# TinfoilHat0/Defending-Against-Backdoors-with-Robust-Learning-Rate

Measured on NVIDIA H100. Metric: fl_rounds_per_sec, higher is better.
Workload: dtype bf16

## Files before the change

defending-against-backdoors-with-robust-learning-rate_b200/models/native.py:

```python
from __future__ import annotations

import math
import os

import torch
import torch.nn.functional as F

from .. import ops
from .graph import FlatLayout

ACT = torch.bfloat16
FUSE_DROPOUT = bool(int(os.environ.get("RLR_FUSE_DROPOUT", "1")))
FUSE_RELU_POOL = bool(int(os.environ.get("RLR_FUSE_RELU_POOL", "1")))
EPILOGUE_BN_STATS = bool(int(os.environ.get("RLR_EPILOGUE_BN_STATS", "0")))
FWD_BRANCH = bool(int(os.environ.get("RLR_FWD_BRANCH", "1")))
BWD_BRANCH = bool(int(os.environ.get("RLR_BWD_BRANCH", "1")))
EPI_STAT_SLOTS = min(16, max(1, int(os.environ.get("RLR_EPI_STAT_SLOTS", "2"))))
FWD_SLOTS = BWD_SLOTS = max(1, int(os.environ.get("RLR_BN_SLOTS", "1")))
WGRAD_OVERLAP = bool(int(os.environ.get("RLR_WGRAD_OVERLAP", "1")))


def dropout_stream_base(seed: int, agent_id: int, rnd: int) -> int:
    z = (int(seed) * 0x9E3779B97F4A7C15 + (int(agent_id) + 1) * 0xBF58476D1CE4E5B9 + (int(rnd) + 1) * 0x94D049BB133111EB) & (2 ** 64 - 1)
    z = ((z ^ (z >> 30)) * 0xBF58476D1CE4E5B9) & (2 ** 64 - 1)
    z = ((z ^ (z >> 27)) * 0x94D049BB133111EB) & (2 ** 64 - 1)
    return (z ^ (z >> 31)) & (2 ** 62 - 1)


def native_supported(layout: FlatLayout) -> bool:
    return all(nd.op in ("conv", "bn", "gn", "relu", "maxpool", "avgpool", "flatten", "dropout", "linear", "save", "add")
               for nd in layout.nodes)


class _Op:
    __slots__ = ("kind", "node", "name", "attrs", "x", "y", "res", "relu", "saved", "acc_dx", "need_dx", "in_shape", "out_shape")

    def __init__(self, kind, **kw):
        self.kind = kind
        self.node = self.name = self.x = self.y = self.res = None
        self.attrs, self.relu, self.saved, self.acc_dx, self.need_dx = {}, False, {}, False, True
        self.in_shape = self.out_shape = None
        for k, v in kw.items():
            setattr(self, k, v)


class NativeNet:
    def __init__(self, layout: FlatLayout, device, max_batch: int, impl: str | dict = "auto", seed: int = 0, act_dtype=None):
        self.layout, self.device, self.max_batch = layout, torch.device(device), int(max_batch)
        self.act_dtype = act_dtype or ACT
        default = ("sm100" if self.device.type == "cuda" else "aten") if impl == "auto" else impl
        self.impl = dict(conv_fwd=default, conv_dgrad=default, conv_wgrad=default, bn=default, pool=default,
                         linear=default, dropout=default) if not isinstance(impl, dict) else dict(impl)
        self.seed = seed
        self.fuse_bn_stats = False
        self.first_wait = None
        self.after_first_op = None
        self.step_counter = torch.zeros(1, dtype=torch.int64, device=device)
        self._build_plan()
        self._alloc()

    def _build_plan(self):
        nodes = self.layout.nodes
        C, H, W = self.layout.in_shape
        shape = {"x": (H, W, C)}
        ver = {"x": 0}
        tid = lambda s: f"{s}@{ver[s]}"
        self.tshape = {tid("x"): shape["x"]}
        plan, consumed = [], set()
        pending_bn = {}
        alias = {}

        def new_out(slot, shp):
            ver[slot] = ver.get(slot, -1) + 1
            shape[slot] = shp
            self.tshape[tid(slot)] = shp
            return tid(slot)

        def next_same_slot(i, slot):
            for j in range(i + 1, len(nodes)):
                if j in consumed:
                    continue
                nd = nodes[j]
                if nd.op == "save":
                    if nd.inp == slot:
                        return None, None
                    continue
                if nd.inp == slot or nd.out == slot:
                    return j, nd
            return None, None

        for i, nd in enumerate(nodes):
            if i in consumed:
                continue
            a = nd.attrs
            if nd.op == "save":
                ver[nd.out] = ver.get(nd.out, -1) + 1
                alias[f"{nd.out}@{ver[nd.out]}"] = tid(nd.inp)
                shape[nd.out] = shape[nd.inp]
                self.tshape[f"{nd.out}@{ver[nd.out]}"] = shape[nd.inp]
                continue
            src = alias.get(tid(nd.inp), tid(nd.inp))
            if nd.op == "conv":
                h, w, c = shape[nd.inp]
                k, s, p = a["k"], a.get("stride", 1), a.get("pad", 0)
                ho, wo = (h + 2 * p - k) // s + 1, (w + 2 * p - k) // s + 1
                op = _Op("conv", node=i, name=nd.name, attrs=a, x=src, in_shape=(h, w, c), out_shape=(ho, wo, a["cout"]))
                j, nx = next_same_slot(i, nd.out)
                want_stats = nx is not None and nx.op == "bn"
                if nx is not None and nx.op == "relu":
                    op.relu = True
                    consumed.add(j)
                op.saved["want_stats"] = want_stats
                op.y = new_out(nd.out, op.out_shape)
                plan.append(op)
            elif nd.op in ("bn", "gn"):
                shp = shape[nd.inp]
                op = _Op(nd.op, node=i, name=nd.name, attrs=a, x=src, in_shape=shp, out_shape=shp)
                j, nx = next_same_slot(i, nd.out)
                if nx is not None and nx.op == "relu":
                    op.relu = True
                    consumed.add(j)
                    op.y = new_out(nd.out, shp)
                    plan.append(op)
                elif nx is not None and nx.op == "add":
                    pending_bn[j] = op
                else:
                    op.y = new_out(nd.out, shp)
                    plan.append(op)
            elif nd.op == "add":
                other = alias.get(tid(a["other"]), tid(a["other"]))
                op = pending_bn.pop(i, None)
                if op is None:
                    raise NotImplementedError("add without a preceding BatchNorm / GroupNorm is not used by any model in the zoo")
                op.res = other
                j, nx = next_same_slot(i, nd.out)
                if nx is not None and nx.op == "relu":
                    op.relu = True
                    consumed.add(j)
                op.y = new_out(nd.out, op.out_shape)
                plan.append(op)
            elif nd.op == "relu":
                raise NotImplementedError("stand-alone ReLU (every ReLU in the zoo follows conv/bn/linear)")
            elif nd.op == "maxpool":
                h, w, c = shape[nd.inp]
                op = _Op("maxpool", node=i, x=src, in_shape=(h, w, c), out_shape=(h // 2, w // 2, c))
                op.y = new_out(nd.out, op.out_shape)
                plan.append(op)
            elif nd.op == "avgpool":
                h, w, c = shape[nd.inp]
                op = _Op("avgpool", node=i, x=src, in_shape=(h, w, c), out_shape=(1, 1, c))
                op.y = new_out(nd.out, op.out_shape)
                plan.append(op)
            elif nd.op == "flatten":
                shp = shape[nd.inp]
                ver[nd.out] += 1
                alias[tid(nd.out)] = src
                shape[nd.out] = (int(math.prod(shp)),)
                self.tshape[tid(nd.out)] = shape[nd.out]
            elif nd.op == "dropout":
                shp = shape[nd.inp]
                prod = next((q for q in reversed(plan) if q.y == src), None)
                fusable = (prod is not None and a.get("p", 0.0) > 0 and "drop" not in prod.saved and
                           (prod.kind == "maxpool" or
                            (prod.kind == "linear" and prod.relu and ops.linear_fused_dropout_ok(prod.attrs["cout"], prod.attrs["cin"]))))
                if fusable and FUSE_DROPOUT:
                    prod.saved["drop"] = (float(a["p"]), i)
                    ver[nd.out] += 1
                    alias[tid(nd.out)] = src
                    shape[nd.out] = shp
                    self.tshape[tid(nd.out)] = shp
                else:
                    op = _Op("dropout", node=i, attrs=a, x=src, in_shape=shp, out_shape=shp)
                    op.y = new_out(nd.out, shp)
                    plan.append(op)
            elif nd.op == "linear":
                op = _Op("linear", node=i, name=nd.name, attrs=a, x=src, in_shape=shape[nd.inp], out_shape=(a["cout"],))
                j, nx = next_same_slot(i, nd.out)
                if nx is not None and nx.op == "relu":
                    op.relu = True
                    consumed.add(j)
                op.y = new_out(nd.out, op.out_shape)
                plan.append(op)
            else:
                raise NotImplementedError(nd.op)
        for op in plan:
            if op.kind != "maxpool":
                continue
            prod = next((q for q in plan if q.y == op.x), None)
            users = [q for q in plan if q.x == op.x or q.res == op.x]
            if prod is not None and prod.kind == "conv" and prod.relu and len(users) == 1 and FUSE_RELU_POOL:
                op.saved["relu_bwd_here"] = True
                prod.saved["relu_bwd_fused"] = True
        self.plan = plan
        self.alias = alias
        self.out_tid = alias.get(tid("x"), tid("x"))
        self.in_tid = "x@0"
        written = set()
        for op in reversed(plan):
            op.need_dx = op.x != self.in_tid
            if op.res is not None:
                written.add(op.res)
            if op.need_dx:
                op.acc_dx = op.x in written
                written.add(op.x)

    def _numel(self, shp):
        return int(math.prod(shp))

    def _alloc(self):
        B, dev = self.max_batch, self.device
        self.act, self.grad = {}, {}
        for op in self.plan:
            self.act[op.y] = torch.empty((B, *op.out_shape), dtype=self.act_dtype, device=dev)
        for op in self.plan:
            for t in (op.x, op.res):
                if t is not None and t != self.in_tid and t not in self.grad:
                    self.grad[t] = torch.empty((B, *self.tshape[t]), dtype=self.act_dtype, device=dev)
        self.grad[self.out_tid] = torch.empty((B, *self.tshape[self.out_tid]), dtype=self.act_dtype, device=dev)
        self.logits = torch.empty((B, self.tshape[self.out_tid][-1]), dtype=torch.float32, device=dev)
        need = [op for op in self.plan if op.kind == "bn" or (op.kind == "conv" and op.saved.get("want_stats"))]
        S = ops.STAT_SLOTS
        tot = sum(2 * op.out_shape[-1] for op in need)
        self.stats_arena = torch.zeros(max(1, tot * S), dtype=torch.float32, device=dev)
        D = BWD_SLOTS
        self.dsum_arena = torch.zeros(max(1, tot * D), dtype=torch.float32, device=dev)
        off = 0
        for op in need:
            c = op.out_shape[-1]
            op.saved["stats"] = self.stats_arena[off * S:(off + 2 * c) * S].view(S, 2, c)
            op.saved["dsum"] = self.dsum_arena[off * D:(off + 2 * c) * D].view(D, 2, c)
            op.saved["mean_rstd"] = torch.zeros(2, c, dtype=torch.float32, device=dev)
            off += 2 * c
        for op in self.plan:
            if op.kind == "gn":
                op.saved["mean_rstd"] = torch.zeros(B, 2, op.attrs["groups"], dtype=torch.float32, device=dev)
            if op.kind == "maxpool":
                op.saved["idx"] = torch.empty((B, *op.out_shape), dtype=torch.uint8, device=dev)
                if "drop" in op.saved and self.impl["pool"] != "sm100":
                    op.saved["dmask"] = torch.ones((B, *op.out_shape), dtype=torch.uint8, device=dev)
            if op.kind == "dropout":
                op.saved["mask"] = torch.empty((B, *op.out_shape), dtype=torch.uint8, device=dev)
        self._bn_src = {}
        for i, op in enumerate(self.plan):
            if not (FWD_BRANCH and op.kind == "conv" and ".downsample." in (op.name or "")):
                continue
            nxt = self.plan[i + 1] if i + 1 < len(self.plan) else None
            first = next((q for q in self.plan[:i] if q.x == op.x and q is not op), None)
            join = next((q for q in self.plan[i + 1:] if nxt is not None and q.res == nxt.y), None)
            if nxt is None or nxt.kind not in ("bn", "gn") or nxt.x != op.y or first is None or join is None:
                continue
            first.saved["fork_before"] = True
            op.saved["side_branch"] = nxt.saved["side_branch"] = True
            join.saved["join_before"] = True
        for i, op in enumerate(self.plan):
            if op.kind == "bn":
                prod = next((q for q in self.plan[:i] if q.y == op.x and q.kind == "conv"), None)
                op.saved["producer"] = prod

    def bind(self, w, wb, g, w_buffers=None):
        self.w, self.wb, self.g = w, wb, g
        lay = self.layout
        self.pw = {p.name: lay.view(w, p) for p in lay.params}
        self.pw.update({b.name: lay.view(w if w_buffers is None else w_buffers, b) for b in lay.buffers})
        self.pwb = {p.name: lay.view(wb, p) for p in lay.params} if wb is not None else {}
        self.pg = {p.name: lay.view(g, p) for p in lay.params} if g is not None else {}

    def T(self, t, B):
        return self.act[t][:B] if t != self.in_tid else self._x

    def stem_geometry(self):
        op = self.plan[0]
        if op.kind != "conv" or op.x != self.in_tid or self.impl["conv_fwd"] != "sm100" or self.impl["conv_wgrad"] != "sm100":
            return None
        return ops.stem_geometry(op.in_shape, op.attrs)

    def G(self, t, B):
        return self.grad[t][:B]

    def forward(self, x_nhwc, train: bool):
        out = self.forward_raw(x_nhwc, train)
        B = out.shape[0]
        self.logits[:B].copy_(out)
        return self.logits[:B]

    def forward_raw(self, x_nhwc, train: bool):
        B = x_nhwc.shape[0] if x_nhwc.dim() == 4 else x_nhwc.shape[0] // (self.plan[0].out_shape[0] * self.plan[0].out_shape[1])
        self._x, self._B, self._train = x_nhwc, B, train
        self._epoch = getattr(self, "_epoch", 0) + 1
        if train:
            ops.zero_(self.stats_arena)
        branch = FWD_BRANCH and self.device.type == "cuda" and ops.nn.USE_STRIDED_TMA and self.impl["conv_fwd"] == "sm100"
        if branch and getattr(self, "_branch_stream", None) is None:
            self._branch_stream = torch.cuda.Stream(self.device)
        for i, op in enumerate(self.plan):
            if branch and op.saved.get("fork_before"):
                self._branch_stream.wait_stream(torch.cuda.current_stream(self.device))
            if branch and op.saved.get("join_before"):
                torch.cuda.current_stream(self.device).wait_stream(self._branch_stream)
            if branch and op.saved.get("side_branch"):
                with torch.cuda.stream(self._branch_stream):
                    getattr(self, "_fwd_" + op.kind)(op, B, train)
            else:
                getattr(self, "_fwd_" + op.kind)(op, B, train)
            if i == 0 and self.after_first_op is not None:
                self.after_first_op()
        return self.T(self.out_tid, B).reshape(B, -1)

    def dlogits_buffer(self, B):
        return self.G(self.out_tid, B).reshape(B, -1)

    def backward(self, dlogits):
        B = dlogits.shape[0]
        gout = self.G(self.out_tid, B)
        if dlogits.data_ptr() != gout.data_ptr():
            gout.copy_(dlogits.reshape(gout.shape))
        ops.zero_(self.g)
        ops.zero_(self.dsum_arena)
        self._side = None
        if WGRAD_OVERLAP and self.device.type == "cuda":
            if getattr(self, "_side_stream", None) is None:
                self._side_stream = torch.cuda.Stream(self.device)
            self._side = self._side_stream
            self._side.wait_stream(torch.cuda.current_stream(self.device))
        branch = (BWD_BRANCH and FWD_BRANCH and self.device.type == "cuda" and ops.nn.USE_STRIDED_TMA and self.impl["conv_fwd"] == "sm100"
                  and getattr(self, "_branch_stream", None) is not None)
        cur = torch.cuda.current_stream(self.device) if branch else None
        for op in reversed(self.plan):
            if branch and op.saved.get("fork_before"):
                cur.wait_stream(self._branch_stream)
            if branch and op.saved.get("side_branch"):
                if op.kind in ("bn", "gn"):
                    self._branch_stream.wait_stream(cur)
                with torch.cuda.stream(self._branch_stream):
                    getattr(self, "_bwd_" + op.kind)(op, B)
            else:
                getattr(self, "_bwd_" + op.kind)(op, B)
        if self._side is not None:
            torch.cuda.current_stream(self.device).wait_stream(self._side)
            self._side = None

    def _epilogue_stats_free(self, op):
        if not EPILOGUE_BN_STATS or self.impl["conv_fwd"] != "sm100":
            return False
        a = op.attrs
        return a.get("stride", 1) == 1 and a["cin"] % 64 == 0 and a["cout"] % 64 == 0 and not (a["k"] == 3 and a["cin"] == 64)

    def _fwd_conv(self, op, B, train):
        a = op.attrs
        x, y = self.T(op.x, B), self.T(op.y, B)
        bias = self.pw.get(op.name + ".bias")
        stats = op.saved.get("stats") if (train and op.saved.get("want_stats") and (self.fuse_bn_stats or self._epilogue_stats_free(op))) else None
        op.saved["stats_done"] = stats is not None
        if self.impl["conv_fwd"] == "sm100" and ops.conv_supported(op.in_shape, a, "fwd"):
            ops.conv2d_fwd_sm100(x, self.pwb[op.name + ".weight"], bias, y, a.get("stride", 1), a.get("pad", 0), op.relu, stats, tag=(id(self), op.name),
                                 zero_stats=False, s2d_epoch=self._epoch, wait=self.first_wait if (op is self.plan[0] and x.dim() == 2) else None)
            return
        if self.impl["conv_fwd"] == "sm100":
            ops.note_fallback("conv_fwd", f"{op.name} in={op.in_shape} {a}")
        wt = self.pwb[op.name + ".weight"].permute(0, 3, 1, 2)
        out = F.conv2d(x.permute(0, 3, 1, 2), wt, bias.to(self.act_dtype) if bias is not None else None, a.get("stride", 1), a.get("pad", 0))
        if op.relu:
            out = F.relu(out)
        y.copy_(out.permute(0, 2, 3, 1))
        if stats is not None:
            yf = y.float().reshape(-1, y.shape[-1])
            stats[0, 0].copy_(yf.sum(0)); stats[0, 1].copy_((yf * yf).sum(0))

    def _bwd_conv(self, op, B):
        a = op.attrs
        x, y, dy = self.T(op.x, B), self.T(op.y, B), self.G(op.y, B)
        if op.relu and not op.saved.get("relu_bwd_fused"):
            ops.relu_bwd_(dy, y, self.impl["bn"])
        name = op.name + ".weight"
        gw, gb = self.pg[name], self.pg.get(op.name + ".bias")
        s, p = a.get("stride", 1), a.get("pad", 0)
        if self.impl["conv_wgrad"] == "sm100" and ops.conv_supported(op.in_shape, a, "wgrad"):
            if getattr(self, "_side", None) is not None:
                self._side.wait_stream(torch.cuda.current_stream(self.device))
                with torch.cuda.stream(self._side):
                    ops.conv2d_wgrad_sm100(x, dy, gw, gb, s, p, tag=(id(self), op.name), zero=False)
            else:
                ops.conv2d_wgrad_sm100(x, dy, gw, gb, s, p, tag=(id(self), op.name), zero=False)
        else:
            if self.impl["conv_wgrad"] == "sm100":
                ops.note_fallback("conv_wgrad", f"{op.name} in={op.in_shape} {a}")
            _, dw, db = torch.ops.aten.convolution_backward(
                dy.permute(0, 3, 1, 2), x.permute(0, 3, 1, 2), self.pwb[name].permute(0, 3, 1, 2),
                [a["cout"]] if gb is not None else None, [s, s], [p, p], [1, 1], False, [0, 0], 1, [False, True, gb is not None])
            gw.copy_(dw.permute(0, 2, 3, 1))
            if gb is not None:
                gb.copy_(db)
        if not op.need_dx:
            return
        dx = self.G(op.x, B)
        if self.impl["conv_dgrad"] == "sm100" and ops.conv_supported(op.in_shape, a, "dgrad"):
            ops.conv2d_dgrad_sm100(dy, self.pwb[name], dx, s, p, op.acc_dx)
            return
        if self.impl["conv_dgrad"] == "sm100":
            ops.note_fallback("conv_dgrad", f"{op.name} in={op.in_shape} {a}")
        di, _, _ = torch.ops.aten.convolution_backward(
            dy.permute(0, 3, 1, 2), x.permute(0, 3, 1, 2), self.pwb[name].permute(0, 3, 1, 2), None, [s, s], [p, p], [1, 1],
            False, [0, 0], 1, [True, False, False])
        di = di.permute(0, 2, 3, 1)
        if op.acc_dx:
            dx.add_(di)
        else:
            dx.copy_(di)

    def _fwd_bn(self, op, B, train):
        a = op.attrs
        x, y = self.T(op.x, B), self.T(op.y, B)
        res = self.T(op.res, B) if op.res is not None else None
        gamma, beta = self.pw[op.name + ".weight"], self.pw[op.name + ".bias"]
        rm, rv = self.pw[op.name + ".running_mean"], self.pw[op.name + ".running_var"]
        prod = op.saved["producer"]
        stats = prod.saved["stats"] if (train and prod is not None and prod.saved.get("stats_done")) else None
        if stats is not None and not self.fuse_bn_stats:
            stats = stats[0:EPI_STAT_SLOTS]
        count = x.numel() // x.shape[-1]
        ops.bn_fwd(x, y, res, gamma, beta, rm, rv, stats, op.saved["mean_rstd"], count, a.get("eps", 1e-5),
                   a.get("momentum", 0.1), train, op.relu, self.impl["bn"],
                   stats_buf=op.saved["stats"][0:FWD_SLOTS] if train else None)

    def _bwd_bn(self, op, B):
        x, y, dy = self.T(op.x, B), self.T(op.y, B), self.G(op.y, B)
        dres = self.G(op.res, B) if op.res is not None else None
        dx = self.G(op.x, B)
        gamma = self.pw[op.name + ".weight"]
        ops.bn_bwd(dy, y, x, gamma, op.saved["mean_rstd"], op.saved["dsum"], dx, dres,
                   self.pg[op.name + ".weight"], self.pg[op.name + ".bias"], op.relu, self.impl["bn"], zero_dsum=False,
                   beta=self.pw[op.name + ".bias"])

    def _fwd_gn(self, op, B, train):
        a = op.attrs
        res = self.T(op.res, B) if op.res is not None else None
        ops.gn_fwd(self.T(op.x, B), self.T(op.y, B), res, self.pw[op.name + ".weight"], self.pw[op.name + ".bias"],
                   op.saved["mean_rstd"][:B], a["groups"], a.get("eps", 1e-5), op.relu, self.impl["bn"])

    def _bwd_gn(self, op, B):
        dres = self.G(op.res, B) if op.res is not None else None
        ops.gn_bwd(self.G(op.y, B), self.T(op.y, B), self.T(op.x, B), self.pw[op.name + ".weight"], op.saved["mean_rstd"][:B],
                   self.G(op.x, B), dres, self.pg[op.name + ".weight"], self.pg[op.name + ".bias"], op.attrs["groups"], op.relu,
                   self.impl["bn"], zero=False)

    def _drop(self, op, train=True):
        d = op.saved.get("drop")
        return (d[0], self.seed, self.step_counter, d[1]) if (d is not None and train) else None

    def _fwd_maxpool(self, op, B, train):
        drop = self._drop(op, train)
        op.saved["drop_on"] = drop is not None
        mask = op.saved["dmask"][:B] if (drop is not None and "dmask" in op.saved) else None
        ops.maxpool2_fwd(self.T(op.x, B), self.T(op.y, B), op.saved["idx"][:B], self.impl["pool"], drop, mask)

    def _bwd_maxpool(self, op, B):
        drop = self._drop(op, op.saved.get("drop_on", False))
        mask = op.saved["dmask"][:B] if (drop is not None and "dmask" in op.saved) else None
        ops.maxpool2_bwd(self.G(op.y, B), op.saved["idx"][:B], self.G(op.x, B), self.impl["pool"], drop, mask,
                         relu_out=self.T(op.y, B) if op.saved.get("relu_bwd_here") else None)

    def _fwd_avgpool(self, op, B, train):
        ops.avgpool_fwd(self.T(op.x, B), self.T(op.y, B), self.impl["pool"])

    def _bwd_avgpool(self, op, B):
        ops.avgpool_bwd(self.G(op.y, B), self.G(op.x, B), self.impl["pool"])

    def _fwd_dropout(self, op, B, train):
        x, y = self.T(op.x, B), self.T(op.y, B)
        if not train:
            y.copy_(x.reshape(y.shape))
            return
        ops.dropout_fwd(x.reshape(B, -1), y.reshape(B, -1), op.saved["mask"][:B].reshape(B, -1), op.attrs["p"], self.seed,
                        self.step_counter, op.node, self.impl["dropout"])

    def _bwd_dropout(self, op, B):
        ops.dropout_bwd(self.G(op.y, B).reshape(B, -1), op.saved["mask"][:B].reshape(B, -1), self.G(op.x, B).reshape(B, -1),
                        op.attrs["p"], self.impl["dropout"])

    def _fwd_linear(self, op, B, train):
        x, y = self.T(op.x, B).reshape(B, -1), self.T(op.y, B)
        drop = self._drop(op, train)
        op.saved["drop_on"] = drop is not None
        ops.linear_fwd(x, self.pwb[op.name + ".weight"], self.pw.get(op.name + ".bias"), y, op.relu, self.impl["linear"], drop)

    def _bwd_linear(self, op, B):
        x, y, dy = self.T(op.x, B).reshape(B, -1), self.T(op.y, B), self.G(op.y, B)
        if op.relu:
            scale = 1.0 / (1.0 - op.saved["drop"][0]) if op.saved.get("drop_on", False) else 1.0
            ops.relu_bwd_(dy, y, self.impl["bn"], scale)
        dx = self.G(op.x, B).reshape(B, -1) if op.need_dx else None
        ops.linear_bwd(x, dy, self.pwb[op.name + ".weight"], dx, self.pg[op.name + ".weight"], self.pg.get(op.name + ".bias"),
                       op.acc_dx, self.impl["linear"], zero=False)


class NativeTrainer:
    name = "native"

    def __init__(self, layout, args, device, max_shard: int, impl="auto"):
        self.layout, self.args = layout, args
        self.device = torch.device(device)
        assert self.device.type == "cuda", "the native trainer runs on sm_90a devices only"
        n = layout.n_total
        self.w = torch.zeros(n, dtype=torch.float32, device=device)
        self.wb = torch.zeros(n, dtype=torch.bfloat16, device=device)
        self.g = torch.zeros(n, dtype=torch.float32, device=device)
        self.m = torch.zeros(n, dtype=torch.float32, device=device)
        self.bs = args.bs
        self.net = NativeNet(layout, device, self.bs, impl, seed=args.seed)
        self.net.bind(self.w, self.wb, self.g)
        self.opt = ops.FlatSGD(n, device, args.client_lr, args.client_moment, 10.0, args.clip, n_pgd=layout.n_vote)
        self.loss_sum = torch.zeros(1, dtype=torch.float32, device=device)
        self.use_graphs = not args.no_graphs
        self.max_shard = max_shard
        self.perm = torch.zeros(max(1, max_shard), dtype=torch.int64, device=device)
        self.cursor = torch.zeros(1, dtype=torch.int32, device=device)
        self.y = torch.zeros(self.bs, dtype=torch.int64, device=device)
        C, H, W = layout.in_shape
        self.x = torch.zeros(self.bs, H, W, C, dtype=ACT, device=device)
        self.stem = self.net.stem_geometry()
        self.xA = torch.zeros(self.bs * self.stem[2] * self.stem[3], 64, dtype=ACT, device=device) if self.stem else None
        self._graphs = {}
        self._eval_nets = {}
        self.bcast = None

    def attach_broadcast(self, fused):
        if self.stem is None or fused.w_bf16 is None:
            return False
        self.bcast = fused
        return True

    def _bind_first(self, w0):
        f = self.bcast
        self.net.bind(f.w_global, f.w_bf16, self.g, w_buffers=self.w)
        lay = self.layout
        first_w = lay.by_name[self.net.plan[0].name + ".weight"]
        lo, hi = f.slices_of(first_w.offset, first_w.offset + first_w.numel)
        self.net.first_wait = (f.ready_ptr, lo, hi, f.epoch_dev) if f.ready_ptr else None
        tail_src, tail_dst = f.w_global[lay.n_vote:], self.w[lay.n_vote:]
        self.net.after_first_op = lambda: ops.ext().acquire_slices(f.ready_ptr, 0, max(0, f.n_slices - 1), f.epoch_dev, tail_src, tail_dst)

    def _bind_normal(self):
        self.net.bind(self.w, self.wb, self.g)
        self.net.first_wait = None
        self.net.after_first_op = None

    def _step(self, dataset, B, w0, first=False):
        if first:
            self._bind_first(w0)
        meta = dataset.meta
        if self.stem is not None:
            k, pad, Ho, Wo = self.stem
            xin = self.xA[:B * Ho * Wo]
            ops.gather_im2col(dataset.data, self.perm, meta.mean, meta.std, k, pad, xin, cursor=self.cursor, targets=dataset.targets,
                              out_labels=self.y, batch=B)
        else:
            xin = self.x[:B]
            ops.gather_normalize(dataset.data, self.perm, meta.mean, meta.std, out=xin, nhwc=True, cursor=self.cursor,
                                 targets=dataset.targets, out_labels=self.y, batch=B)
        logits = self.net.forward_raw(xin, True)
        _, dl = ops.softmax_xent(logits, self.y[:B], True, self.loss_sum, dlogits=self.net.dlogits_buffer(B))
        self.net.backward(dl)
        self.opt.step(self.w, self.g, self.m, w0=w0, w_bf16=self.wb, w_in=self.bcast.w_global if first else None)
        ops.ext().advance_cursor(self.cursor, B, self.net.step_counter)
        if first:
            self._bind_normal()

    def _get_graph(self, dataset, B, w0, first=False):
        key = (B, dataset.data.data_ptr(), w0.data_ptr(), bool(first))
        if key in self._graphs:
            return self._graphs[key]
        keep = (self.w.clone(), self.wb.clone(), self.m.clone(), self.cursor.clone(), self.loss_sum.clone(),
                self.net.step_counter.clone())
        self.perm.zero_()
        s = torch.cuda.Stream(self.device)
        s.wait_stream(torch.cuda.current_stream(self.device))
        with torch.cuda.stream(s):
            for _ in range(3):
                self.cursor.zero_()
                c0 = ops.launch_calls()
                self._step(dataset, B, w0, first)
                self._launches = ops.launch_calls() - c0
        torch.cuda.current_stream(self.device).wait_stream(s)
        self.cursor.zero_()
        graph = torch.cuda.CUDAGraph()
        with torch.cuda.graph(graph, capture_error_mode="thread_local"):
            self._step(dataset, B, w0, first)
        self.w.copy_(keep[0]); self.wb.copy_(keep[1]); self.m.copy_(keep[2]); self.cursor.copy_(keep[3])
        self.loss_sum.copy_(keep[4]); self.net.step_counter.copy_(keep[5])
        self._graphs[key] = graph
        return graph

    def train_agent(self, agent, w_global, out, rnd: int = 0):
        args, bs = self.args, self.bs
        dataset, n = agent.dataset, agent.n_data
        self.loss_sum.zero_()
        graphs = self.use_graphs and n <= self.max_shard
        fused = self.bcast is not None and w_global.data_ptr() == self.bcast.w_global.data_ptr()
        if graphs:
            full = self._get_graph(dataset, bs, w_global) if n >= bs else None
            tail = self._get_graph(dataset, n % bs, w_global) if n % bs else None
            if fused:
                first_g = self._get_graph(dataset, bs if n >= bs else n % bs, w_global, first=True)
        if not fused:
            ops.round_init(w_global, self.w, self.wb, self.m)
        self.net.step_counter.fill_(dropout_stream_base(args.seed, agent.id, rnd))
        steps = 0
        for ep in range(args.local_ep):
            idx = agent.epoch_indices(args.seed, rnd, ep)
            self.perm[:n].copy_(idx)
            self.cursor.zero_()
            for b in range(n // bs):
                is_first = fused and ep == 0 and b == 0
                if graphs:
                    (first_g if is_first else full).replay()
                else:
                    self._step(dataset, bs, w_global, first=is_first)
            if n % bs:
                is_first = fused and ep == 0 and n < bs
                if graphs:
                    (first_g if is_first else tail).replay()
                else:
                    self._step(dataset, n % bs, w_global, first=is_first)
            steps += (n + bs - 1) // bs
        if out.data_ptr() != self.w.data_ptr():
            out.copy_(self.w)
        return {"loss_sum": self.loss_sum, "steps": steps}

    def launches_per_step(self):
        return getattr(self, "_launches", 0)

    @torch.no_grad()
    def eval_forward(self, w):
        key = w.data_ptr()
        if key not in self._eval_nets:
            net = NativeNet(self.layout, self.device, self.bs, self.net.impl, seed=self.args.seed)
            self._eval_nets = {key: (net, torch.zeros(self.layout.n_total, dtype=ACT, device=self.device))}
        net, wb = self._eval_nets[key]
        wb.copy_(w)
        net.bind(w, wb, None)

        def fwd(x_nchw):
            x = x_nchw.permute(0, 2, 3, 1).to(ACT).contiguous()
            return net.forward(x, False).clone()
        return fwd
```

defending-against-backdoors-with-robust-learning-rate_b200/ops/csrc/gemm.cu:

```cuda
#include <cuda.h>
#include <stdlib.h>

#include "common.cuh"
#include "gemm.h"
#include "stem_gather.cuh"
#include "wgmma.cuh"

namespace rlr {

using namespace wg;

constexpr int BM = 128;
constexpr int BK = 64;
constexpr int kConsumers = 256;
constexpr int kThreads = kConsumers + 64;
constexpr int kEpiThreads = kConsumers;

template <int BN, int kOcc = 2>
struct TileCfg {
    static constexpr int kStages = kOcc == 3 ? (BN == 64 ? 3 : 2) : (BN == 64 ? 4 : 3);
    static constexpr int kABytes = BM * BK * 2;
    static constexpr int kBBytes = BN * BK * 2;
    static constexpr int kStageBytes = kABytes + kBBytes;
    static constexpr int kPitch = BN * 2 + 16;
    static constexpr int kStagingBytes = BM * kPitch;
    static constexpr int kRingBytes = kStages * kStageBytes;
    static_assert(kStagingBytes + 2 * BN * 4 <= kRingBytes, "staging aliases the operand ring");
    static constexpr int kTailBytes = BN == 128 ? 2048 : 1024;
    static constexpr int kSmemBytes = kRingBytes + 1024  + kTailBytes;
};

struct __align__(8) SharedTail {
    uint64_t full[4];
    uint64_t empty[4];
    uint64_t pad0;
    uint32_t pad1;
    uint32_t pad2;
    int row_index[BM];
};
static_assert(sizeof(SharedTail) <= 640, "the bias slice starts 640 bytes into the tail");

template <int BN, bool kStats, bool kBMN, int kOcc = 2>
__global__ void __launch_bounds__(kThreads, kOcc)
umma_conv_gemm_kernel(const __grid_constant__ CUtensorMap tmA, const __grid_constant__ CUtensorMap tmB, const __grid_constant__ CUtensorMap tmC,
                       const ConvGemmParams p) {
    using Cfg = TileCfg<BN, kOcc>;
    extern __shared__ uint8_t smem_raw[];
    uint8_t* smem = reinterpret_cast<uint8_t*>((reinterpret_cast<uintptr_t>(smem_raw) + 1023) & ~uintptr_t(1023));
    SharedTail* tail = reinterpret_cast<SharedTail*>(smem + Cfg::kRingBytes);

    const int warp = threadIdx.x >> 5, lane = threadIdx.x & 31;
    const int tile_m = blockIdx.x, tile_n = blockIdx.y;
    long long* dbg = p.dbg ? p.dbg + ((size_t)blockIdx.y * gridDim.x + blockIdx.x) * 8 : nullptr;
    if (dbg && threadIdx.x == 0) { dbg[0] = (long long)gtimer(); uint32_t sm; asm volatile("mov.u32 %0, %%smid;" : "=r"(sm)); dbg[7] = sm; }

    int n0 = 0, h0 = 0, w0 = 0;
    if (p.mode == 1) {
        const int tw_i = tile_m % p.tiles_w;
        const int th_i = (tile_m / p.tiles_w) % p.tiles_h;
        const int tn_i = tile_m / (p.tiles_w * p.tiles_h);
        w0 = tw_i * p.TW; h0 = th_i * p.TH; n0 = tn_i * p.TN;
    }

    if (warp == 8 && lane == 0) {
        prefetch_tmap(&tmA);
        prefetch_tmap(&tmB);
        if (p.tma_store) prefetch_tmap(&tmC);
        for (int s = 0; s < Cfg::kStages; ++s) { mbar_init(&tail->full[s], (p.split_prod || p.b_src) ? 2 : 1); mbar_init(&tail->empty[s], 8); }
        fence_barrier_init();
    }
    if (threadIdx.x < BM) {
        const int r = threadIdx.x;
        int gi;
        if (p.mode == 1) {
            const int tw = r % p.TW, th = (r / p.TW) % p.TH, tn = r / (p.TW * p.TH);
            const int w = w0 + tw, h = h0 + th, n = n0 + tn;
            gi = (w < p.Wo && h < p.Ho && n < p.NB) ? ((n * p.OutH + h * p.out_stride + p.out_ph) * p.OutW + w * p.out_stride + p.out_pw) : -1;
        } else {
            gi = tile_m * BM + r;
            if (gi >= p.M) gi = -1;
        }
        tail->row_index[r] = gi;
    }
    __syncthreads();
    pdl_wait();
    pdl_trigger();
    if (dbg && threadIdx.x == 0) dbg[1] = (long long)gtimer();

    if (warp == 8) {
        if (p.b_src) {
            if (lane == 0) {
                mbar_expect_tx(&tail->full[0], Cfg::kABytes);
                tma_load_2d(&tmA, &tail->full[0], smem, 0, tile_m * BM);
            }
            stem_gather_b(p, smem + Cfg::kABytes, BN, tile_n, lane);
            if (lane == 0) mbar_arrive(&tail->full[0]);
        } else if (lane == 0) {
            int stage = 0;
            uint32_t phase = 0;
            for (int kb = 0; kb < p.num_kb; ++kb) {
                mbar_wait(&tail->empty[stage], phase ^ 1);
                uint8_t* sa = smem + stage * Cfg::kStageBytes;
                uint8_t* sb = sa + Cfg::kABytes;
                mbar_expect_tx(&tail->full[stage], p.split_prod ? Cfg::kABytes : Cfg::kStageBytes);
                if (dbg && kb == 0) dbg[2] = (long long)gtimer();
                if (p.mode == 1) {
                    const int tap = kb / p.cblocks, cb = kb - tap * p.cblocks;
                    tma_load_4d(&tmA, &tail->full[stage], sa, cb * BK, w0 * p.in_stride + p.dw[tap], h0 * p.in_stride + p.dh[tap],
                                n0 + p.dn[tap]);
                } else {
                    tma_load_2d(&tmA, &tail->full[stage], sa, kb * BK, tile_m * BM);
                }
                if (p.split_prod) {
                } else if (kBMN) {
                    const int tap = kb / p.cblocks, cb = kb - tap * p.cblocks;
                    for (int g = 0; g < BN / 64; ++g)
                        tma_load_2d(&tmB, &tail->full[stage], sb + g * 8192, p.wtap[tap] * p.wcols + tile_n * BN + g * 64, cb * BK);
                } else {
                    tma_load_2d(&tmB, &tail->full[stage], sb, kb * BK, tile_n * BN);
                }
                if (++stage == Cfg::kStages) { stage = 0; phase ^= 1; }
            }
        }
    } else if (warp == 9) {
        if (p.split_prod && lane == 0) {
            int stage = 0;
            uint32_t phase = 0;
            for (int kb = 0; kb < p.num_kb; ++kb) {
                mbar_wait(&tail->empty[stage], phase ^ 1);
                uint8_t* sb = smem + stage * Cfg::kStageBytes + Cfg::kABytes;
                mbar_expect_tx(&tail->full[stage], Cfg::kBBytes);
                if (kBMN) {
                    const int tap = kb / p.cblocks, cb = kb - tap * p.cblocks;
                    for (int g = 0; g < BN / 64; ++g)
                        tma_load_2d(&tmB, &tail->full[stage], sb + g * 8192, p.wtap[tap] * p.wcols + tile_n * BN + g * 64, cb * BK);
                } else {
                    tma_load_2d(&tmB, &tail->full[stage], sb, kb * BK, tile_n * BN);
                }
                if (++stage == Cfg::kStages) { stage = 0; phase ^= 1; }
            }
        }
    } else {
        const int et = threadIdx.x;
        const int wgi = et >> 7, t = et & 127;
        const int col0 = tile_n * BN;
        const bool has_bias = !kBMN && p.bias != nullptr;
        float* bias_w = reinterpret_cast<float*>(reinterpret_cast<uint8_t*>(tail) + 640);
        if (has_bias)
            for (int i = et; i < BN; i += kEpiThreads) bias_w[i] = (col0 + i < p.N) ? p.bias[col0 + i] : 0.f;
        float acc[BN / 2];
#pragma unroll
        for (int i = 0; i < BN / 2; ++i) acc[i] = 0.f;
        {
            int stage = 0;
            uint32_t phase = 0;
            consumer_mainloop<BN, Cfg::kStages, Cfg::kStageBytes, Cfg::kABytes, kBMN>(
                acc, smem, tail->full, tail->empty, p.num_kb, (uint32_t)wgi * 64 * 128, p.b_src ? smem_u32(smem + Cfg::kABytes) : 0u,
                stage, phase, lane);
        }
        if (dbg && et == 0) dbg[4] = (long long)gtimer();
        named_bar(1, kEpiThreads);
        if (dbg && et == 0) dbg[5] = (long long)gtimer();
        const float* bias_s = bias_w;
        uint8_t* staging = smem;
        float* red = reinterpret_cast<float*>(staging + Cfg::kStagingBytes);
        const int r0 = wgi * 64 + frag_row(t, 0);
        int gi_r[2];
        gi_r[0] = tail->row_index[r0];
        gi_r[1] = tail->row_index[r0 + 8];
        if (kStats) {
            for (int i = et; i < 2 * BN; i += kEpiThreads) red[i] = 0.f;
            named_bar(1, kEpiThreads);
        }
        const bool tma_out = !kStats && p.tma_store;
#pragma unroll
        for (int j = 0; j < BN / 8; ++j) {
            const int c = frag_col(t, 4 * j);
            float s1[2] = {0.f, 0.f}, s2[2] = {0.f, 0.f};
#pragma unroll
            for (int h = 0; h < 2; ++h) {
                const int row = r0 + 8 * h, gi_row = gi_r[h];
                float a = acc[4 * j + 2 * h], b = acc[4 * j + 2 * h + 1];
                if (has_bias) { a += bias_s[c]; b += bias_s[c + 1]; }
                if (p.relu) { a = fmaxf(a, 0.f); b = fmaxf(b, 0.f); }
                if (p.drop.thr) {
                    const uint32_t keep8 = dropout_keep8(p.drop, ((long long)(gi_row < 0 ? 0 : gi_row) * p.ldc + col0 + 8 * j) >> 3);
                    a = (keep8 >> (c & 7) & 1) ? a * p.drop.scale : 0.f;
                    b = (keep8 >> ((c & 7) + 1) & 1) ? b * p.drop.scale : 0.f;
                }
                const uint32_t packed = pack_bf16x2(a, b);
                if (kStats && gi_row >= 0) {
                    const float2 rq = __bfloat1622float2(*reinterpret_cast<const __nv_bfloat162*>(&packed));
                    s1[0] += rq.x; s1[1] += rq.y; s2[0] += rq.x * rq.x; s2[1] += rq.y * rq.y;
                }
                if (tma_out)
                    *reinterpret_cast<uint32_t*>(staging + (c >> 6) * (BM * 128) + row * 128 + ((((c & 63) >> 3) ^ (row & 7)) << 4) + (c & 7) * 2) = packed;
                else
                    *reinterpret_cast<uint32_t*>(staging + row * Cfg::kPitch + c * 2) = packed;
            }
            if (kStats) {
#pragma unroll
                for (int o = 4; o < 32; o <<= 1)
#pragma unroll
                    for (int e = 0; e < 2; ++e) {
                        s1[e] += __shfl_xor_sync(0xffffffffu, s1[e], o);
                        s2[e] += __shfl_xor_sync(0xffffffffu, s2[e], o);
                    }
                if (lane < 4) {
                    atomicAdd(&red[c], s1[0]); atomicAdd(&red[c + 1], s1[1]);
                    atomicAdd(&red[BN + c], s2[0]); atomicAdd(&red[BN + c + 1], s2[1]);
                }
            }
        }
        if (tma_out) {
            fence_proxy_async_smem();
            named_bar(1, kEpiThreads);
            if (dbg && et == 0) dbg[6] = (long long)gtimer();
            if (et == 0) {
#pragma unroll
                for (int g = 0; g < BN / 64; ++g) {
                    if (col0 + g * 64 >= p.N) break;
                    if (p.mode == 1) tma_store_4d(&tmC, staging + g * (BM * 128), col0 + g * 64, w0, h0, n0);
                    else tma_store_2d(&tmC, staging + g * (BM * 128), col0 + g * 64, tile_m * BM);
                }
                tma_store_commit();
            }
            if (p.stats) {
                constexpr int kPerCol = kEpiThreads / BN, kRows = BM / kPerCol;
                const int c = et % BN;
                const int r_lo = (et / BN) * kRows, r_hi = r_lo + kRows;
                const uint8_t* colp = staging + (c >> 6) * (BM * 128) + (c & 7) * 2;
                const int chunk = (c & 63) >> 3;
                float s1 = 0.f, s2 = 0.f;
#pragma unroll 8
                for (int r = r_lo; r < r_hi; ++r) {
                    if (tail->row_index[r] < 0) continue;
                    const float v = __bfloat162float(*reinterpret_cast<const __nv_bfloat16*>(colp + r * 128 + ((chunk ^ (r & 7)) << 4)));
                    s1 += v; s2 += v * v;
                }
                if (col0 + c < p.N) {
                    float* dst = p.stats + (size_t)(blockIdx.x % p.stat_slots) * 2 * p.N + col0 + c;
                    atomicAdd(dst, s1);
                    atomicAdd(dst + p.N, s2);
                }
            }
            if (et == 0) tma_store_wait_read();
        } else {
        named_bar(1, kEpiThreads);
        if (dbg && et == 0) dbg[6] = (long long)gtimer();
        constexpr int kChunks = BN * 2 / 16;
        __nv_bfloat16* out = reinterpret_cast<__nv_bfloat16*>(p.out);
        constexpr int kIters = BM * kChunks / kEpiThreads;
        constexpr int kBatch = kIters < 8 ? kIters : 8;
#pragma unroll
        for (int it0 = 0; it0 < kIters; it0 += kBatch) {
            uint4 oldv[kBatch];
            if (p.accumulate) {
#pragma unroll
                for (int j = 0; j < kBatch; ++j) {
                    const int idx = et + (it0 + j) * kEpiThreads, r = idx / kChunks, ch = idx - r * kChunks;
                    const int gi = tail->row_index[r];
                    oldv[j] = make_uint4(0, 0, 0, 0);
                    if (gi >= 0 && col0 + ch * 8 < p.N) oldv[j] = *reinterpret_cast<const uint4*>(out + (size_t)gi * p.ldc + col0 + ch * 8);
                }
            }
#pragma unroll
            for (int j = 0; j < kBatch; ++j) {
                const int idx = et + (it0 + j) * kEpiThreads, r = idx / kChunks, ch = idx - r * kChunks;
                const int gi = tail->row_index[r];
                if (gi < 0 || col0 + ch * 8 >= p.N) continue;
                uint4 val = *reinterpret_cast<const uint4*>(staging + r * Cfg::kPitch + ch * 16);
                if (p.accumulate) {
                    const __nv_bfloat162* o2 = reinterpret_cast<const __nv_bfloat162*>(&oldv[j]);
                    __nv_bfloat162* v2 = reinterpret_cast<__nv_bfloat162*>(&val);
#pragma unroll
                    for (int q = 0; q < 4; ++q) {
                        const float2 a = __bfloat1622float2(v2[q]), b = __bfloat1622float2(o2[q]);
                        v2[q] = __floats2bfloat162_rn(a.x + b.x, a.y + b.y);
                    }
                }
                *reinterpret_cast<uint4*>(out + (size_t)gi * p.ldc + col0 + ch * 8) = val;
            }
        }
        if (kStats) {
            named_bar(1, kEpiThreads);
            for (int i = et; i < 2 * BN; i += kEpiThreads)
                if (col0 + (i % BN) < p.N)
                    atomicAdd(p.stats + (size_t)(blockIdx.x % kStatSlots) * 2 * p.N + (i < BN ? 0 : p.N) + col0 + (i % BN), red[i]);
        }
        }
    }
}

typedef CUresult (*EncodeTiledFn)(CUtensorMap*, CUtensorMapDataType, cuuint32_t, void*, const cuuint64_t*, const cuuint64_t*,
                                  const cuuint32_t*, const cuuint32_t*, CUtensorMapInterleave, CUtensorMapSwizzle,
                                  CUtensorMapL2promotion, CUtensorMapFloatOOBfill);

static EncodeTiledFn get_encode_fn() {
    static EncodeTiledFn fn = nullptr;
    if (!fn) {
        void* f = nullptr;
        cudaDriverEntryPointQueryResult q;
        if (cudaGetDriverEntryPoint("cuTensorMapEncodeTiled", &f, cudaEnableDefault, &q) != cudaSuccess || !f) return nullptr;
        fn = reinterpret_cast<EncodeTiledFn>(f);
    }
    return fn;
}

cudaError_t make_tmap_bf16(CUtensorMap* map, const void* base, int rank, const uint64_t* dims, const uint64_t* strides_bytes,
                           const uint32_t* box, const uint32_t* elem_strides = nullptr) {
    EncodeTiledFn fn = get_encode_fn();
    if (!fn) return cudaErrorNotSupported;
    cuuint64_t gd[5], gs[4];
    cuuint32_t bx[5], es[5];
    for (int i = 0; i < rank; ++i) {
        gd[i] = dims[i];
        es[i] = elem_strides ? elem_strides[i] : 1;
        bx[i] = box[i] * es[i];
        if (bx[i] > 256 || es[i] < 1 || es[i] > 8) return cudaErrorInvalidValue;
    }
    for (int i = 0; i + 1 < rank; ++i) gs[i] = strides_bytes[i];
    const CUresult r = fn(map, CU_TENSOR_MAP_DATA_TYPE_BFLOAT16, (cuuint32_t)rank, const_cast<void*>(base), gd, gs, bx, es,
                          CU_TENSOR_MAP_INTERLEAVE_NONE, CU_TENSOR_MAP_SWIZZLE_128B, CU_TENSOR_MAP_L2_PROMOTION_L2_256B,
                          CU_TENSOR_MAP_FLOAT_OOB_FILL_NONE);
    return r == CUDA_SUCCESS ? cudaSuccess : cudaErrorInvalidValue;
}

template <int BN>
cudaError_t launch_persistent_bn(const CUtensorMap& tmA, const CUtensorMap& tmB, const ConvGemmParams& p, int m_tiles, int num_sms,
                                 cudaStream_t st, int occ = 1);

static int g_occ3 = -1;
void set_conv_occ3(int level) { g_occ3 = level < 0 ? 0 : (level > 1 ? 1 : level); }
static int conv_occ3() {
    if (g_occ3 < 0) { const char* e = getenv("RLR_CONV_OCC3"); set_conv_occ3(e ? atoi(e) : 1); }
    return g_occ3;
}

template <int BN>
static cudaError_t launch_bn_occ3(const CUtensorMap& tmA, const CUtensorMap& tmB, const CUtensorMap& tmC, const ConvGemmParams& p, int m_tiles,
                                  cudaStream_t st) {
    using Cfg = TileCfg<BN, 3>;
    static bool configured = false;
    if (!configured) {
        RLR_CUDA_CHECK(cudaFuncSetAttribute(umma_conv_gemm_kernel<BN, false, false, 3>, cudaFuncAttributeMaxDynamicSharedMemorySize, Cfg::kSmemBytes));
        RLR_CUDA_CHECK(cudaFuncSetAttribute(umma_conv_gemm_kernel<BN, false, true, 3>, cudaFuncAttributeMaxDynamicSharedMemorySize, Cfg::kSmemBytes));
        configured = true;
    }
    dim3 grid(m_tiles, (p.N + BN - 1) / BN);
    if (p.b_mn) return launch_kernel(umma_conv_gemm_kernel<BN, false, true, 3>, grid, dim3(kThreads), Cfg::kSmemBytes, st, tmA, tmB, tmC, p);
    return launch_kernel(umma_conv_gemm_kernel<BN, false, false, 3>, grid, dim3(kThreads), Cfg::kSmemBytes, st, tmA, tmB, tmC, p);
}

static int sm_count() {
    static const int sms = [] {
        int dev = 0, n = 0;
        if (cudaGetDevice(&dev) != cudaSuccess || cudaDeviceGetAttribute(&n, cudaDevAttrMultiProcessorCount, dev) != cudaSuccess) return 132;
        return n;
    }();
    return sms;
}

static int g_persistent = -1;
void set_persistent_conv(int on) { g_persistent = on ? 1 : 0; }

static int persistent_sms() {
    if (g_persistent < 0) { const char* e = getenv("RLR_PERSISTENT_CONV"); g_persistent = (e && atoi(e) > 0) ? 1 : 0; }
    if (!g_persistent) return 0;
    static const int sms = [] {
        int dev = 0, n = 0;
        if (cudaGetDevice(&dev) != cudaSuccess || cudaDeviceGetAttribute(&n, cudaDevAttrMultiProcessorCount, dev) != cudaSuccess) return 0;
        return n;
    }();
    return sms;
}

static int g_split_prod = -1;
void set_conv_split_producer(int on) { g_split_prod = on ? 1 : 0; }
static long long* g_trace = nullptr;
void set_conv_trace(long long* buf) { g_trace = buf; }
long long* conv_trace_buf() { return g_trace; }

static int g_tma_store = -1;
void set_conv_tma_store(int on) { g_tma_store = on ? 1 : 0; }
static bool tma_store_enabled() {
    if (g_tma_store < 0) { const char* e = getenv("RLR_TMA_STORE"); g_tma_store = (e && atoi(e) == 0) ? 0 : 1; }
    return g_tma_store != 0;
}
static cudaError_t make_out_tmap(CUtensorMap* tmC, const ConvGemmParams& p) {
    if (p.ldc % 8) return cudaErrorInvalidValue;
    if (p.mode == 1) {
        const uint64_t d[4] = {(uint64_t)p.N, (uint64_t)p.Wo, (uint64_t)p.Ho, (uint64_t)p.NB};
        const uint64_t s[3] = {(uint64_t)p.out_stride * p.ldc * 2, (uint64_t)p.out_stride * p.OutW * p.ldc * 2, (uint64_t)p.OutH * p.OutW * p.ldc * 2};
        const uint32_t b[4] = {64, (uint32_t)p.TW, (uint32_t)p.TH, (uint32_t)p.TN};
        const char* base = reinterpret_cast<const char*>(p.out) + ((size_t)p.out_ph * p.OutW + p.out_pw) * p.ldc * 2;
        return make_tmap_bf16(tmC, base, 4, d, s, b);
    }
    const uint64_t d[2] = {(uint64_t)p.N, (uint64_t)p.M}, s[1] = {(uint64_t)p.ldc * 2};
    const uint32_t b[2] = {64, BM};
    return make_tmap_bf16(tmC, p.out, 2, d, s, b);
}

template <int BN>
static cudaError_t launch_bn(const CUtensorMap& tmA, const CUtensorMap& tmB, const ConvGemmParams& p_in, int m_tiles, cudaStream_t st) {
    using Cfg = TileCfg<BN>;
    ConvGemmParams p = p_in;
    p.dbg = g_trace;
    CUtensorMap tmC = tmA;
    {
        static const int epi_slots = [] { const char* e = getenv("RLR_EPI_STAT_SLOTS"); int v = e ? atoi(e) : 2; return v < 1 ? 1 : (v > kStatSlots ? kStatSlots : v); }();
        p.stat_slots = epi_slots;
    }
    p.tma_store = 0;
    if (tma_store_enabled() && !p.accumulate && ((reinterpret_cast<uintptr_t>(p.out) & 15) == 0) && make_out_tmap(&tmC, p) == cudaSuccess)
        p.tma_store = 1;
    if (g_split_prod < 0) { const char* e = getenv("RLR_SPLIT_PRODUCER"); g_split_prod = (e && atoi(e) == 0) ? 0 : 1; }
    p.split_prod = (g_split_prod && !p.b_src) ? 1 : 0;
    if (p.b_src && !p.stats && p.N <= BN) {
        static const int stem_persistent = [] { const char* e = getenv("RLR_STEM_PERSISTENT"); return e ? atoi(e) : 2; }();
        if (stem_persistent && m_tiles >= 2 * sm_count())
            return launch_persistent_bn<BN>(tmA, tmB, p, m_tiles, sm_count(), st, stem_persistent == 2 ? 2 : 1);
    }
    if (!p.stats && !p.b_src && persistent_sms() > 0 && m_tiles * ((p.N + BN - 1) / BN) > persistent_sms())
        return launch_persistent_bn<BN>(tmA, tmB, p, m_tiles, persistent_sms(), st);
    if constexpr (BN == 64)
        if ((!p.stats || p.tma_store) && conv_occ3() >= 1) return launch_bn_occ3<BN>(tmA, tmB, tmC, p, m_tiles, st);
    static bool configured = false;
    if (!configured) {
        RLR_CUDA_CHECK(cudaFuncSetAttribute(umma_conv_gemm_kernel<BN, false, false>, cudaFuncAttributeMaxDynamicSharedMemorySize, Cfg::kSmemBytes));
        RLR_CUDA_CHECK(cudaFuncSetAttribute(umma_conv_gemm_kernel<BN, true, false>, cudaFuncAttributeMaxDynamicSharedMemorySize, Cfg::kSmemBytes));
        RLR_CUDA_CHECK(cudaFuncSetAttribute(umma_conv_gemm_kernel<BN, false, true>, cudaFuncAttributeMaxDynamicSharedMemorySize, Cfg::kSmemBytes));
        configured = true;
    }
    dim3 grid(m_tiles, (p.N + BN - 1) / BN);
    if (p.b_mn) return launch_kernel(umma_conv_gemm_kernel<BN, false, true>, grid, dim3(kThreads), Cfg::kSmemBytes, st, tmA, tmB, tmC, p);
    if (p.stats && !p.tma_store) return launch_kernel(umma_conv_gemm_kernel<BN, true, false>, grid, dim3(kThreads), Cfg::kSmemBytes, st, tmA, tmB, tmC, p);
    return launch_kernel(umma_conv_gemm_kernel<BN, false, false>, grid, dim3(kThreads), Cfg::kSmemBytes, st, tmA, tmB, tmC, p);
}

static int pick_bn(int N) { return (N % 128 == 0) ? 128 : 64; }

cudaError_t launch_gemm_bf16(const void* A, const void* B, void* out, int M, int N, int K, int lda, int ldb, int ldc,
                             const float* bias, int relu, int accumulate, float* stats, cudaStream_t st, const DropSpec* drop) {
    if (K % BK || N % 8 || M <= 0) return cudaErrorInvalidValue;
    if (drop && drop->thr && (accumulate || stats || ldc % 8)) return cudaErrorInvalidValue;
    const int m_tiles = (M + BM - 1) / BM;
    int bn = pick_bn(N);
    {
        static const int small64 = [] { const char* e = getenv("RLR_GEMM_SMALL_BN64"); return e ? atoi(e) : 0; }();
        if (small64 && bn == 128 && m_tiles * (N / 128) < sm_count()) bn = 64;
    }
    CUtensorMap tmA, tmB;
    {
        const uint64_t d[2] = {(uint64_t)K, (uint64_t)M}, s[1] = {(uint64_t)lda * 2};
        const uint32_t b[2] = {BK, BM};
        RLR_CUDA_CHECK(make_tmap_bf16(&tmA, A, 2, d, s, b));
    }
    {
        const uint64_t d[2] = {(uint64_t)K, (uint64_t)N}, s[1] = {(uint64_t)ldb * 2};
        const uint32_t b[2] = {BK, (uint32_t)bn};
        RLR_CUDA_CHECK(make_tmap_bf16(&tmB, B, 2, d, s, b));
    }
    ConvGemmParams p{};
    p.M = M; p.N = N; p.num_kb = K / BK; p.mode = 0; p.in_stride = 1; p.out_stride = 1;
    p.out = out; p.ldc = ldc; p.bias = bias; p.stats = stats; p.relu = relu; p.accumulate = accumulate;
    if (drop && drop->thr) p.drop = *drop;
    return bn == 128 ? launch_bn<128>(tmA, tmB, p, m_tiles, st) : launch_bn<64>(tmA, tmB, p, m_tiles, st);
}

cudaError_t launch_stem_gemm_bf16(const void* A, const void* W, void* out, int M, int N, int kvalid, int ldw, const float* bias, int relu,
                                  float* stats, const uint32_t* wait_flags, int wait_lo, int wait_hi, const uint32_t* wait_epoch,
                                  cudaStream_t st) {
    if (N % 8 || M <= 0 || kvalid < 1 || kvalid > BK || ldw < kvalid) return cudaErrorInvalidValue;
    if (wait_flags && (!wait_epoch || wait_lo > wait_hi || wait_lo < 0)) return cudaErrorInvalidValue;
    const int m_tiles = (M + BM - 1) / BM;
    const int bn = pick_bn(N);
    CUtensorMap tmA;
    {
        const uint64_t d[2] = {(uint64_t)BK, (uint64_t)M}, s[1] = {(uint64_t)BK * 2};
        const uint32_t b[2] = {BK, BM};
        RLR_CUDA_CHECK(make_tmap_bf16(&tmA, A, 2, d, s, b));
    }
    ConvGemmParams p{};
    p.M = M; p.N = N; p.num_kb = 1; p.mode = 0; p.in_stride = 1; p.out_stride = 1;
    p.out = out; p.ldc = N; p.bias = bias; p.stats = stats; p.relu = relu; p.accumulate = 0;
    p.b_src = reinterpret_cast<const __nv_bfloat16*>(W); p.b_ld = ldw; p.b_kvalid = kvalid;
    p.wait_flags = wait_flags; p.wait_lo = wait_lo; p.wait_hi = wait_hi; p.wait_epoch = wait_epoch;
    return bn == 128 ? launch_bn<128>(tmA, tmA, p, m_tiles, st) : launch_bn<64>(tmA, tmA, p, m_tiles, st);
}

static int pow2_ceil(int x) { int p = 1; while (p < x) p <<= 1; return p; }

cudaError_t launch_conv_bf16(const void* x, const void* w, void* out, int NB, int planes, int Hin, int Win, int Cin, int Ho, int Wo,
                             int Cout, int ldc, int ntaps, const int* dh, const int* dw, const int* dplane, const float* bias,
                             int relu, int accumulate, float* stats, cudaStream_t st, const int* wtap, int w_taps_total,
                             int in_stride, int out_stride, int out_ph, int out_pw) {
    if (Cin % BK || Cout % 8 || ntaps < 1 || ntaps > 9) return cudaErrorInvalidValue;
    if (in_stride < 1 || in_stride > 2 || out_stride < 1 || out_stride > 2 || (in_stride > 1 && planes != 1)) return cudaErrorInvalidValue;
    if (wtap && (stats || Cout % 64)) return cudaErrorInvalidValue;
    int bn = pick_bn(Cout);
    ConvGemmParams p{};
    {
        static const int small_bn64 = [] { const char* e = getenv("RLR_SMALL_BN64"); return e ? atoi(e) : 1; }();
        const long long px = (long long)NB * Ho * Wo;
        if (small_bn64 && bn == 128 && ((px + BM - 1) / BM) * (Cout / 128) < sm_count()) bn = 64;
    }
    int TW = pow2_ceil(Wo); if (TW > BM) TW = BM;
    int TH = pow2_ceil(Ho); if (TW * TH > BM) TH = BM / TW;
    int TN = BM / (TW * TH);
    p.TW = TW; p.TH = TH; p.TN = TN;
    p.tiles_w = (Wo + TW - 1) / TW; p.tiles_h = (Ho + TH - 1) / TH;
    const int tiles_n = (NB + TN - 1) / TN;
    const int m_tiles = p.tiles_w * p.tiles_h * tiles_n;
    p.M = NB * Ho * Wo; p.N = Cout; p.mode = 1; p.cblocks = Cin / BK; p.num_kb = ntaps * p.cblocks; p.ntaps = ntaps;
    p.Ho = Ho; p.Wo = Wo; p.NB = NB;
    p.in_stride = in_stride; p.out_stride = out_stride; p.out_ph = out_ph; p.out_pw = out_pw; p.OutH = Ho * out_stride; p.OutW = Wo * out_stride;
    for (int t = 0; t < ntaps; ++t) { p.dh[t] = (int8_t)dh[t]; p.dw[t] = (int8_t)dw[t]; p.dn[t] = dplane[t] * NB; }
    p.out = out; p.ldc = ldc; p.bias = bias; p.stats = stats; p.relu = relu; p.accumulate = accumulate;
    CUtensorMap tmA, tmB;
    {
        const uint64_t d[4] = {(uint64_t)Cin, (uint64_t)Win, (uint64_t)Hin, (uint64_t)planes * NB};
        const uint64_t s[3] = {(uint64_t)Cin * 2, (uint64_t)Win * Cin * 2, (uint64_t)Hin * Win * Cin * 2};
        const uint32_t b[4] = {BK, (uint32_t)TW, (uint32_t)TH, (uint32_t)TN};
        const uint32_t es[4] = {1, (uint32_t)in_stride, (uint32_t)in_stride, 1};
        RLR_CUDA_CHECK(make_tmap_bf16(&tmA, x, 4, d, s, b, in_stride > 1 ? es : nullptr));
    }
    if (wtap) {
        if (bias) return cudaErrorInvalidValue;
        p.b_mn = 1; p.wcols = Cout;
        for (int t = 0; t < ntaps; ++t) p.wtap[t] = wtap[t];
        const uint64_t cols = (uint64_t)w_taps_total * Cout;
        const uint64_t d[2] = {cols, (uint64_t)Cin}, s[1] = {cols * 2};
        const uint32_t b[2] = {64, BK};
        RLR_CUDA_CHECK(make_tmap_bf16(&tmB, w, 2, d, s, b));
    } else {
        const uint64_t K = (uint64_t)ntaps * Cin;
        const uint64_t d[2] = {K, (uint64_t)Cout}, s[1] = {K * 2};
        const uint32_t b[2] = {BK, (uint32_t)bn};
        RLR_CUDA_CHECK(make_tmap_bf16(&tmB, w, 2, d, s, b));
    }
    return bn == 128 ? launch_bn<128>(tmA, tmB, p, m_tiles, st) : launch_bn<64>(tmA, tmB, p, m_tiles, st);
}

}
```

defending-against-backdoors-with-robust-learning-rate_b200/ops/csrc/gemm.h:

```cpp
#pragma once
#include <cuda_runtime.h>
#include <cuda_bf16.h>
#include <stdint.h>

#include "dropspec.h"

namespace rlr {

constexpr int kStatSlots = 16;

struct ConvGemmParams {
    int M, N, num_kb;
    int mode;
    int cblocks;
    int TW, TH, TN;
    int Ho, Wo, NB;
    int tiles_w, tiles_h;
    int ntaps;
    int in_stride;
    int out_stride, out_ph, out_pw, OutH, OutW;
    int8_t dh[9], dw[9];
    int dn[9];
    int b_mn;
    int wtap[9];
    int wcols;
    DropSpec drop;
    int tma_store;
    int split_prod;
    long long* dbg;
    const __nv_bfloat16* b_src;
    int b_ld, b_kvalid;
    const uint32_t* wait_flags;
    int wait_lo, wait_hi;
    const uint32_t* wait_epoch;
    void* out;
    int ldc;
    const float* bias;
    float* stats;
    int stat_slots;
    int relu, accumulate;
};

cudaError_t launch_gemm_bf16(const void* A, const void* B, void* out, int M, int N, int K, int lda, int ldb, int ldc,
                             const float* bias, int relu, int accumulate, float* stats, cudaStream_t st, const DropSpec* drop = nullptr);
cudaError_t launch_stem_gemm_bf16(const void* A, const void* W, void* out, int M, int N, int kvalid, int ldw, const float* bias, int relu,
                                  float* stats, const uint32_t* wait_flags, int wait_lo, int wait_hi, const uint32_t* wait_epoch,
                                  cudaStream_t st);
void set_pdl(int on);
cudaError_t launch_gemm_splitk_bf16(const void* A, const void* B, void* out, float* ws, int M, int N, int K, const float* bias, int relu,
                                    int num_sms, cudaStream_t st, const DropSpec* drop = nullptr);
void set_persistent_conv(int on);
void set_conv_occ3(int level);
void set_conv_tma_store(int on);
void set_conv_split_producer(int on);
void set_conv_trace(long long* buf);
long long* conv_trace_buf();
cudaError_t launch_conv_bf16(const void* x, const void* w, void* out, int NB, int planes, int Hin, int Win, int Cin, int Ho, int Wo,
                             int Cout, int ldc, int ntaps, const int* dh, const int* dw, const int* dplane, const float* bias,
                             int relu, int accumulate, float* stats, cudaStream_t st, const int* wtap = nullptr, int w_taps_total = 0,
                             int in_stride = 1, int out_stride = 1, int out_ph = 0, int out_pw = 0);

cudaError_t launch_conv3x3_halo_bf16(const void* x, const void* w, void* out, int NB, int Hin, int Win, int H, int W, int Cout, const float* bias,
                                     int relu, int accumulate, float* stats, int bo_mode, long long* dbg, int num_sms, cudaStream_t st);

cudaError_t launch_conv3x3_halo3_bf16(const void* x, const void* w, void* out, int NB, int H, int W, int Cout, const float* bias, int relu,
                                      int accumulate, int num_sms, cudaStream_t st);

cudaError_t launch_conv_wgrad_bf16(const void* dy, const void* x, float* dW, int NB, int planes, int Hin, int Win, int Cin, int Cin_valid,
                                   int Ho, int Wo, int Cout, int ntaps, const int* dh, const int* dw, const int* dplane, int num_sms,
                                   cudaStream_t st, int in_stride = 1);
cudaError_t launch_conv_wgrad_halo_bf16(const void* dy, const void* x, float* dW, int NB, int H, int W, int Cin_valid, int Cout,
                                        int num_sms, cudaStream_t st);
cudaError_t launch_linear_wgrad_bf16(const void* dy, const void* x, float* dW, int B, int N, int K, int num_sms, cudaStream_t st);

cudaError_t launch_ordered_sum_f32(float* out, const float* part, int nparts, long long n, cudaStream_t st);
cudaError_t launch_ordered_sum_f64(double* out, const double* part, int nparts, long long n, cudaStream_t st);
cudaError_t launch_channel_stats(const __nv_bfloat16* x, long long M, int C, float* stats , int num_sms, cudaStream_t st,
                                 int only_sum = 0, int nslots = 1);
cudaError_t launch_bn_finalize(const float* stats, int slots, float* mean_rstd, float* running_mean, float* running_var, int C,
                               float count, float eps, float momentum, int train, cudaStream_t st);
cudaError_t launch_bn_apply(const __nv_bfloat16* x, const __nv_bfloat16* res, __nv_bfloat16* y, const float* gamma, const float* beta,
                            float* mean_rstd, long long M, int C, int relu, int fin_mode, const float* stats, int slots, float count,
                            float eps, float momentum, float* running_mean, float* running_var, int num_sms, cudaStream_t st);
cudaError_t launch_bn_bwd_reduce(const __nv_bfloat16* dy, const __nv_bfloat16* y, const __nv_bfloat16* x, const float* mean_rstd,
                                 float* dsum , long long M, int C, int relu, int num_sms, cudaStream_t st,
                                 const float* gamma = nullptr, const float* beta = nullptr, int nslots = 1);
cudaError_t launch_bn_bwd_apply(const __nv_bfloat16* dy, const __nv_bfloat16* y, const __nv_bfloat16* x, const float* gamma,
                                const float* mean_rstd, const float* dsum, __nv_bfloat16* dx, __nv_bfloat16* dres, float* dgamma,
                                float* dbeta, long long M, int C, int relu, int num_sms, cudaStream_t st, const float* beta = nullptr, int nslots = 1);
cudaError_t launch_gn_fwd(const __nv_bfloat16* x, const __nv_bfloat16* res, __nv_bfloat16* y, const float* gamma, const float* beta,
                          float* mean_rstd, int B, int HW, int C, int G, float eps, int relu, int num_sms, cudaStream_t st);
cudaError_t launch_gn_bwd(const __nv_bfloat16* dy, const __nv_bfloat16* y, const __nv_bfloat16* x, const float* gamma,
                          const float* mean_rstd, __nv_bfloat16* dx, __nv_bfloat16* dres, float* dgamma, float* dbeta, int B, int HW,
                          int C, int G, int relu, int num_sms, cudaStream_t st);
cudaError_t launch_relu_bwd(__nv_bfloat16* dy, const __nv_bfloat16* y, long long n, int num_sms, cudaStream_t st, float scale = 1.0f);
cudaError_t launch_maxpool2_fwd(const __nv_bfloat16* x, __nv_bfloat16* y, uint8_t* idx, int B, int H, int W, int C, cudaStream_t st,
                                float drop_p = 0.f, uint64_t seed = 0, const long long* step = nullptr, uint64_t stream = 0);
cudaError_t launch_maxpool2_bwd(const __nv_bfloat16* dy, const uint8_t* idx, __nv_bfloat16* dx, int B, int H, int W, int C, cudaStream_t st,
                                float drop_p, uint64_t seed, const long long* step, uint64_t stream, const __nv_bfloat16* zmask);
cudaError_t launch_avgpool_fwd(const __nv_bfloat16* x, __nv_bfloat16* y, int B, int HW, int C, cudaStream_t st);
cudaError_t launch_avgpool_bwd(const __nv_bfloat16* dy, __nv_bfloat16* dx, int B, int HW, int C, cudaStream_t st);
cudaError_t launch_dropout_fwd(const __nv_bfloat16* x, __nv_bfloat16* y, uint8_t* mask, long long n, float p, uint64_t seed,
                               const long long* step, uint64_t stream, cudaStream_t st);
cudaError_t launch_dropout_bwd(const __nv_bfloat16* dy, const uint8_t* mask, __nv_bfloat16* dx, long long n, float p, cudaStream_t st);
cudaError_t launch_space_to_depth(const __nv_bfloat16* x, __nv_bfloat16* y, int NB, int H, int W, int C, int num_sms, cudaStream_t st);
cudaError_t launch_im2col_small(const __nv_bfloat16* x, __nv_bfloat16* A, int NB, int H, int W, int C, int Ho, int Wo, int k, int pad,
                                int num_sms, cudaStream_t st);
cudaError_t launch_depth_to_space(const __nv_bfloat16* x4, __nv_bfloat16* y, int NB, int H, int W, int C, int accumulate, int plane_mask,
                                  int num_sms, cudaStream_t st);
cudaError_t launch_filter_gather_transpose(const __nv_bfloat16* w, __nv_bfloat16* wt, int Cout, int T, int Cin, int nsub, const int* taps,
                                           cudaStream_t st);
cudaError_t launch_filter_transpose(const __nv_bfloat16* w, __nv_bfloat16* wt, int Cout, int ntaps, int Cin, cudaStream_t st);
cudaError_t launch_linear_small_fwd(const __nv_bfloat16* x, const __nv_bfloat16* w, const float* bias, __nv_bfloat16* y, int B, int K,
                                    int N, int relu, cudaStream_t st);
cudaError_t launch_linear_small_fwd2(const __nv_bfloat16* x, const __nv_bfloat16* w, const float* bias, __nv_bfloat16* y, int B, int K,
                                     int N, int relu, cudaStream_t st);
cudaError_t launch_linear_small_bwd2(const __nv_bfloat16* x, const __nv_bfloat16* dy, const __nv_bfloat16* w, __nv_bfloat16* dx,
                                     float* dw, float* db, int B, int K, int N, int accumulate_dx, cudaStream_t st);
cudaError_t launch_linear_small_bwd(const __nv_bfloat16* x, const __nv_bfloat16* dy, const __nv_bfloat16* w, __nv_bfloat16* dx,
                                    float* dw, float* db, int B, int K, int N, int accumulate_dx, cudaStream_t st);

}
```

defending-against-backdoors-with-robust-learning-rate_b200/ops/csrc/gemm_binding.cpp:

```cpp
#include <torch/extension.h>
#include <ATen/cuda/CUDAContext.h>
#include <c10/cuda/CUDAGuard.h>
#include <c10/cuda/CUDAStream.h>
#include <c10/cuda/CUDACachingAllocator.h>

#include <vector>

#include "gemm.h"

namespace rlr {
void* scratch_alloc(size_t bytes, cudaStream_t st) {
    return c10::cuda::CUDACachingAllocator::raw_alloc_with_stream(bytes < 256 ? 256 : bytes, st);
}
void scratch_free(void* p) { c10::cuda::CUDACachingAllocator::raw_delete(p); }
}

namespace {
inline cudaStream_t cur_stream() { return c10::cuda::getCurrentCUDAStream().stream(); }
inline int num_sms() { return at::cuda::getCurrentDeviceProperties()->multiProcessorCount; }
inline void check(cudaError_t e, const char* what) { TORCH_CHECK(e == cudaSuccess, what, ": ", cudaGetErrorString(e)); }
template <typename T>
inline T* opt(const c10::optional<at::Tensor>& t) { return t.has_value() && t->defined() ? reinterpret_cast<T*>(t->data_ptr()) : nullptr; }
inline const __nv_bfloat16* bf(const at::Tensor& t) {
    TORCH_CHECK(t.is_cuda() && t.scalar_type() == at::kBFloat16 && t.is_contiguous(), "expected contiguous CUDA bf16 tensor");
    return reinterpret_cast<const __nv_bfloat16*>(t.data_ptr());
}
inline __nv_bfloat16* bfm(at::Tensor& t) { return const_cast<__nv_bfloat16*>(bf(t)); }
inline const __nv_bfloat16* bfo(const c10::optional<at::Tensor>& t) { return t.has_value() && t->defined() ? bf(*t) : nullptr; }
inline float* f32(const at::Tensor& t) {
    TORCH_CHECK(t.is_cuda() && t.scalar_type() == at::kFloat && t.is_contiguous(), "expected contiguous CUDA fp32 tensor");
    return reinterpret_cast<float*>(t.data_ptr());
}

static rlr::DropSpec drop_spec(double p, int64_t seed, const c10::optional<at::Tensor>& step, int64_t stream) {
    rlr::DropSpec d{};
    if (p > 0.0) {
        TORCH_CHECK(p < 1.0 && step.has_value() && step->defined() && step->scalar_type() == at::kLong, "fused dropout needs p < 1 and an int64 step counter");
        d.thr = (uint32_t)(p * 65536.0); d.scale = (float)(1.0 / (1.0 - p)); d.seed = (uint64_t)seed; d.stream = (uint64_t)stream;
        d.step = reinterpret_cast<const long long*>(step->data_ptr<int64_t>());
    }
    return d;
}

void gemm_bf16(at::Tensor A, at::Tensor B, at::Tensor out, c10::optional<at::Tensor> bias, bool relu, bool accumulate,
               c10::optional<at::Tensor> stats, double drop_p, int64_t drop_seed, c10::optional<at::Tensor> drop_step, int64_t drop_stream) {
    c10::cuda::CUDAGuard g(A.device());
    const rlr::DropSpec drop = drop_spec(drop_p, drop_seed, drop_step, drop_stream);
    const int M = A.size(0), K = A.size(1), N = B.size(0);
    TORCH_CHECK(B.size(1) == K && out.size(0) == M && out.size(1) == N);
    TORCH_CHECK(!stats.has_value() || !stats->defined() || stats->numel() == (int64_t)rlr::kStatSlots * 2 * N, "stats must be [STAT_SLOTS,2,N]");
    check(rlr::launch_gemm_bf16(bf(A), bf(B), bfm(out), M, N, K, K, K, N, opt<const float>(bias), relu, accumulate, opt<float>(stats),
                                cur_stream(), drop.thr ? &drop : nullptr), "gemm_bf16");
}

void stem_gemm_bf16(at::Tensor A, at::Tensor W, at::Tensor out, c10::optional<at::Tensor> bias, bool relu, c10::optional<at::Tensor> stats,
                    int64_t ready_ptr, int64_t lo, int64_t hi, c10::optional<at::Tensor> epoch) {
    c10::cuda::CUDAGuard g(A.device());
    const int M = A.size(0), N = W.size(0), kvalid = W.size(1);
    TORCH_CHECK(A.dim() == 2 && A.size(1) == 64 && W.dim() == 2 && W.is_contiguous() && out.size(0) == M && out.size(1) == N, "stem_gemm shapes");
    TORCH_CHECK(ready_ptr == 0 || (epoch.has_value() && epoch->defined() && epoch->scalar_type() == at::kInt), "epoch must be an int32 device tensor");
    check(rlr::launch_stem_gemm_bf16(bf(A), bf(W), bfm(out), M, N, kvalid, kvalid, opt<const float>(bias), relu, opt<float>(stats),
                                     reinterpret_cast<const uint32_t*>(ready_ptr), (int)lo, (int)hi,
                                     ready_ptr ? reinterpret_cast<const uint32_t*>(epoch->data_ptr()) : nullptr, cur_stream()), "stem_gemm_bf16");
}

void conv_bf16(at::Tensor x, at::Tensor w, at::Tensor out, int64_t NB, int64_t planes, std::vector<int64_t> dh, std::vector<int64_t> dw,
               std::vector<int64_t> dplane, c10::optional<at::Tensor> bias, bool relu, bool accumulate, c10::optional<at::Tensor> stats,
               std::vector<int64_t> wtap, int64_t w_taps_total) {
    c10::cuda::CUDAGuard g(x.device());
    TORCH_CHECK(x.dim() == 4 && out.dim() == 4 && w.dim() == 2);
    const int Hin = x.size(1), Win = x.size(2), Cin = x.size(3), Ho = out.size(1), Wo = out.size(2), Cout = out.size(3);
    const int T = (int)dh.size();
    const bool bmn = !wtap.empty();
    TORCH_CHECK(x.size(0) == planes * NB && out.size(0) == NB);
    TORCH_CHECK(bmn ? (w.size(0) == Cin && w.size(1) == w_taps_total * Cout && (int)wtap.size() == T)
                    : (w.size(0) == Cout && w.size(1) == (int64_t)T * Cin), "filter shape");
    TORCH_CHECK(!stats.has_value() || !stats->defined() || stats->numel() == (int64_t)rlr::kStatSlots * 2 * Cout, "stats must be [STAT_SLOTS,2,Cout]");
    int a[9], b[9], c[9], wt[9];
    for (int t = 0; t < T; ++t) { a[t] = (int)dh[t]; b[t] = (int)dw[t]; c[t] = (int)dplane[t]; wt[t] = bmn ? (int)wtap[t] : 0; }
    check(rlr::launch_conv_bf16(bf(x), bf(w), bfm(out), (int)NB, (int)planes, Hin, Win, Cin, Ho, Wo, Cout, Cout, T, a, b, c,
                                opt<const float>(bias), relu, accumulate, opt<float>(stats), cur_stream(), bmn ? wt : nullptr,
                                (int)w_taps_total), "conv_bf16");
}

void gemm_splitk_bf16(at::Tensor A, at::Tensor B, at::Tensor out, at::Tensor ws, c10::optional<at::Tensor> bias, bool relu, double drop_p,
                      int64_t drop_seed, c10::optional<at::Tensor> drop_step, int64_t drop_stream) {
    c10::cuda::CUDAGuard g(A.device());
    const rlr::DropSpec drop = drop_spec(drop_p, drop_seed, drop_step, drop_stream);
    const int M = A.size(0), K = A.size(1), N = B.size(0);
    TORCH_CHECK(B.size(1) == K && out.size(0) == M && out.size(1) == N && ws.numel() == (int64_t)M * N);
    check(rlr::launch_gemm_splitk_bf16(bf(A), bf(B), bfm(out), f32(ws), M, N, K, opt<const float>(bias), relu, num_sms(), cur_stream(),
                                       drop.thr ? &drop : nullptr), "gemm_splitk_bf16");
}

void conv_bf16_strided(at::Tensor x, at::Tensor w, at::Tensor out, std::vector<int64_t> dh, std::vector<int64_t> dw,
                       c10::optional<at::Tensor> bias, bool relu, bool accumulate, std::vector<int64_t> wtap, int64_t w_taps_total,
                       int64_t in_stride, int64_t out_stride, int64_t out_ph, int64_t out_pw) {
    c10::cuda::CUDAGuard g(x.device());
    TORCH_CHECK(x.dim() == 4 && out.dim() == 4 && w.dim() == 2 && x.size(0) == out.size(0));
    TORCH_CHECK(out.size(1) % out_stride == 0 && out.size(2) % out_stride == 0, "output image must be a multiple of out_stride");
    const int NB = x.size(0), Hin = x.size(1), Win = x.size(2), Cin = x.size(3), Cout = out.size(3);
    const int Ho = out.size(1) / out_stride, Wo = out.size(2) / out_stride;
    const int T = (int)dh.size();
    const bool bmn = !wtap.empty();
    TORCH_CHECK(bmn ? (w.size(0) == Cin && w.size(1) == w_taps_total * Cout && (int)wtap.size() == T)
                    : (w.size(0) == Cout && w.size(1) == (int64_t)T * Cin), "filter shape");
    int a[9], b[9], c[9] = {0}, wt[9];
    for (int t = 0; t < T; ++t) { a[t] = (int)dh[t]; b[t] = (int)dw[t]; wt[t] = bmn ? (int)wtap[t] : 0; }
    check(rlr::launch_conv_bf16(bf(x), bf(w), bfm(out), NB, 1, Hin, Win, Cin, Ho, Wo, Cout, Cout, T, a, b, c, opt<const float>(bias), relu,
                                accumulate, nullptr, cur_stream(), bmn ? wt : nullptr, (int)w_taps_total, (int)in_stride, (int)out_stride,
                                (int)out_ph, (int)out_pw), "conv_bf16_strided");
}

void conv3x3_halo_bf16(at::Tensor x, at::Tensor w, at::Tensor out, c10::optional<at::Tensor> bias, bool relu, bool accumulate,
                       c10::optional<at::Tensor> stats, int64_t bo_mode, c10::optional<at::Tensor> dbg) {
    c10::cuda::CUDAGuard g(x.device());
    TORCH_CHECK(x.dim() == 4 && x.size(3) == 64 && out.dim() == 4 && w.dim() == 2 && w.size(1) == 9 * 64 && w.size(0) == out.size(3));
    TORCH_CHECK(out.size(0) == x.size(0) && out.size(1) - x.size(1) == out.size(2) - x.size(2), "halo conv: output = input + 2*pad - 2, pad in {0,1,2}");
    TORCH_CHECK(!stats.has_value() || !stats->defined() || stats->numel() == (int64_t)rlr::kStatSlots * 2 * out.size(3), "stats must be [STAT_SLOTS,2,Cout]");
    check(rlr::launch_conv3x3_halo_bf16(bf(x), bf(w), bfm(out), x.size(0), x.size(1), x.size(2), out.size(1), out.size(2), out.size(3), opt<const float>(bias), relu,
                                        accumulate, opt<float>(stats), (int)bo_mode, opt<long long>(dbg), num_sms(), cur_stream()), "conv3x3_halo_bf16");
}

void conv3x3_halo3_bf16(at::Tensor x, at::Tensor w, at::Tensor out, c10::optional<at::Tensor> bias, bool relu, bool accumulate) {
    c10::cuda::CUDAGuard g(x.device());
    TORCH_CHECK(x.dim() == 4 && x.size(3) == 64 && out.dim() == 4 && w.dim() == 2 && w.size(1) == 9 * 64 && w.size(0) == out.size(3));
    TORCH_CHECK(out.size(0) == x.size(0) && out.size(1) == x.size(1) && out.size(2) == x.size(2));
    check(rlr::launch_conv3x3_halo3_bf16(bf(x), bf(w), bfm(out), x.size(0), x.size(1), x.size(2), out.size(3), opt<const float>(bias), relu,
                                         accumulate, num_sms(), cur_stream()), "conv3x3_halo3_bf16");
}

void conv_wgrad_bf16(at::Tensor dy, at::Tensor x, at::Tensor dW, int64_t NB, int64_t planes, int64_t cin_valid, std::vector<int64_t> dh,
                     std::vector<int64_t> dw, std::vector<int64_t> dplane) {
    c10::cuda::CUDAGuard g(x.device());
    TORCH_CHECK(x.dim() == 4 && dy.dim() == 4);
    const int Hin = x.size(1), Win = x.size(2), Cin = x.size(3), Ho = dy.size(1), Wo = dy.size(2), Cout = dy.size(3);
    const int T = (int)dh.size();
    TORCH_CHECK(x.size(0) == planes * NB && dy.size(0) == NB && dW.numel() == (int64_t)Cout * T * cin_valid);
    TORCH_CHECK((Cout <= 64 && Cout % 8 == 0) || Cout % 128 == 0, "wgrad: Cout must be <= 64 or a multiple of 128");
    int a[9], b[9], c[9];
    for (int t = 0; t < T; ++t) { a[t] = (int)dh[t]; b[t] = (int)dw[t]; c[t] = (int)dplane[t]; }
    check(rlr::launch_conv_wgrad_bf16(bf(dy), bf(x), f32(dW), (int)NB, (int)planes, Hin, Win, Cin, (int)cin_valid, Ho, Wo, Cout, T, a, b, c,
                                      num_sms(), cur_stream()), "conv_wgrad_bf16");
}
void conv_wgrad_bf16_strided(at::Tensor dy, at::Tensor x, at::Tensor dW, int64_t cin_valid, std::vector<int64_t> dh, std::vector<int64_t> dw,
                             int64_t in_stride) {
    c10::cuda::CUDAGuard g(x.device());
    TORCH_CHECK(x.dim() == 4 && dy.dim() == 4 && x.size(0) == dy.size(0));
    const int NB = x.size(0), Hin = x.size(1), Win = x.size(2), Cin = x.size(3), Ho = dy.size(1), Wo = dy.size(2), Cout = dy.size(3);
    const int T = (int)dh.size();
    TORCH_CHECK(dW.numel() == (int64_t)Cout * T * cin_valid);
    TORCH_CHECK((Cout <= 64 && Cout % 8 == 0) || Cout % 128 == 0, "wgrad: Cout must be <= 64 or a multiple of 128");
    int a[9], b[9], c[9] = {0};
    for (int t = 0; t < T; ++t) { a[t] = (int)dh[t]; b[t] = (int)dw[t]; }
    check(rlr::launch_conv_wgrad_bf16(bf(dy), bf(x), f32(dW), NB, 1, Hin, Win, Cin, (int)cin_valid, Ho, Wo, Cout, T, a, b, c, num_sms(),
                                      cur_stream(), (int)in_stride), "conv_wgrad_bf16_strided");
}
void conv_wgrad_halo_bf16(at::Tensor dy, at::Tensor x, at::Tensor dW, int64_t cin_valid) {
    c10::cuda::CUDAGuard g(x.device());
    TORCH_CHECK(x.dim() == 4 && x.size(3) == 64 && dy.dim() == 4 && dy.size(0) == x.size(0) && dy.size(1) == x.size(1) && dy.size(2) == x.size(2));
    TORCH_CHECK(dW.numel() == dy.size(3) * 9 * cin_valid);
    check(rlr::launch_conv_wgrad_halo_bf16(bf(dy), bf(x), f32(dW), x.size(0), x.size(1), x.size(2), (int)cin_valid, dy.size(3), num_sms(),
                                           cur_stream()), "conv_wgrad_halo_bf16");
}
void linear_wgrad_bf16(at::Tensor dy, at::Tensor x, at::Tensor dW) {
    c10::cuda::CUDAGuard g(x.device());
    const int B = x.size(0), K = x.size(1), N = dy.size(1);
    TORCH_CHECK(dy.size(0) == B && dW.numel() == (int64_t)N * K && ((N <= 64 && N % 8 == 0) || N % 128 == 0));
    check(rlr::launch_linear_wgrad_bf16(bf(dy), bf(x), f32(dW), B, N, K, num_sms(), cur_stream()), "linear_wgrad_bf16");
}

void ordered_sum(at::Tensor out, at::Tensor part) {
    c10::cuda::CUDAGuard g(out.device());
    TORCH_CHECK(out.is_contiguous() && part.is_contiguous() && part.dim() == 2 && part.size(1) == out.numel() &&
                part.scalar_type() == out.scalar_type(), "ordered_sum: out [n], part [nparts][n]");
    const int nparts = (int)part.size(0);
    const long long n = out.numel();
    if (out.scalar_type() == at::kDouble)
        check(rlr::launch_ordered_sum_f64(out.data_ptr<double>(), part.data_ptr<double>(), nparts, n, cur_stream()), "ordered_sum");
    else
        check(rlr::launch_ordered_sum_f32(out.data_ptr<float>(), part.data_ptr<float>(), nparts, n, cur_stream()), "ordered_sum");
}

void channel_stats(at::Tensor x, at::Tensor stats) {
    c10::cuda::CUDAGuard g(x.device());
    const int C = x.size(-1);
    const int nslots = (int)(stats.numel() / (2 * C));
    TORCH_CHECK(nslots >= 1 && stats.numel() == (int64_t)nslots * 2 * C, "stats must be [slots, 2, C]");
    check(rlr::launch_channel_stats(bf(x), x.numel() / C, C, f32(stats), num_sms(), cur_stream(), 0, nslots), "channel_stats");
}
void bias_grad(at::Tensor dy, at::Tensor db) {
    c10::cuda::CUDAGuard g(dy.device());
    const int C = dy.size(-1);
    TORCH_CHECK(db.numel() == C && db.scalar_type() == at::kFloat && dy.is_contiguous(), "bias_grad: db must be fp32 [C]");
    check(rlr::launch_channel_stats(bf(dy), dy.numel() / C, C, f32(db), num_sms(), cur_stream(), 1), "bias_grad");
}
void bn_finalize(at::Tensor stats, at::Tensor mean_rstd, at::Tensor rm, at::Tensor rv, double count, double eps, double momentum, bool train) {
    c10::cuda::CUDAGuard g(stats.device());
    const int C = mean_rstd.size(-1);
    const int slots = (int)(stats.numel() / (2 * C));
    TORCH_CHECK(slots >= 1 && stats.numel() == (int64_t)slots * 2 * C, "stats must be [slots, 2, C]");
    check(rlr::launch_bn_finalize(f32(stats), slots, f32(mean_rstd), (float*)rm.data_ptr(), (float*)rv.data_ptr(), C, (float)count, (float)eps,
                                  (float)momentum, train, cur_stream()), "bn_finalize");
}
void bn_apply(at::Tensor x, c10::optional<at::Tensor> res, at::Tensor y, at::Tensor gamma, at::Tensor beta, at::Tensor mean_rstd, bool relu,
              int64_t fin_mode, c10::optional<at::Tensor> stats, double count, double eps, double momentum,
              c10::optional<at::Tensor> rm, c10::optional<at::Tensor> rv) {
    c10::cuda::CUDAGuard g(x.device());
    const int C = x.size(-1);
    int slots = 1;
    if (fin_mode == 1) {
        TORCH_CHECK(stats.has_value() && stats->defined() && rm.has_value() && rv.has_value(), "bn_apply: training finalize needs stats and running stats");
        slots = (int)(stats->numel() / (2 * C));
        TORCH_CHECK(slots >= 1 && stats->numel() == (int64_t)slots * 2 * C, "stats must be [slots,2,C]");
    }
    if (fin_mode == 2) TORCH_CHECK(rm.has_value() && rv.has_value(), "bn_apply: eval needs running stats");
    check(rlr::launch_bn_apply(bf(x), bfo(res), bfm(y), (const float*)gamma.data_ptr(), (const float*)beta.data_ptr(), f32(mean_rstd),
                               x.numel() / C, C, relu, (int)fin_mode, opt<const float>(stats), slots, (float)count, (float)eps, (float)momentum,
                               opt<float>(rm), opt<float>(rv), num_sms(), cur_stream()), "bn_apply");
}
void bn_bwd(at::Tensor dy, at::Tensor y, at::Tensor x, at::Tensor gamma, at::Tensor mean_rstd, at::Tensor dsum, at::Tensor dx,
            c10::optional<at::Tensor> dres, at::Tensor dgamma, at::Tensor dbeta, bool relu, bool zero_dsum) {
    c10::cuda::CUDAGuard g(x.device());
    const int C = x.size(-1);
    const long long M = x.numel() / C;
    const int nslots = (int)(dsum.numel() / (2 * C));
    TORCH_CHECK(nslots >= 1 && dsum.numel() == (int64_t)nslots * 2 * C, "dsum must be [slots, 2, C]");
    if (zero_dsum) check(cudaMemsetAsync(dsum.data_ptr(), 0, sizeof(float) * dsum.numel(), cur_stream()), "bn_bwd/memset");
    check(rlr::launch_bn_bwd_reduce(bf(dy), bf(y), bf(x), f32(mean_rstd), f32(dsum), M, C, relu, num_sms(), cur_stream(), nullptr, nullptr, nslots),
          "bn_bwd_reduce");
    check(rlr::launch_bn_bwd_apply(bf(dy), bf(y), bf(x), (const float*)gamma.data_ptr(), f32(mean_rstd), f32(dsum), bfm(dx),
                                   const_cast<__nv_bfloat16*>(bfo(dres)), (float*)dgamma.data_ptr(), (float*)dbeta.data_ptr(), M, C, relu,
                                   num_sms(), cur_stream(), nullptr, nslots), "bn_bwd_apply");
}
void bn_bwd_recompute(at::Tensor dy, at::Tensor x, at::Tensor gamma, at::Tensor beta, at::Tensor mean_rstd, at::Tensor dsum, at::Tensor dx,
                      at::Tensor dgamma, at::Tensor dbeta, bool zero_dsum) {
    c10::cuda::CUDAGuard g(x.device());
    const int C = x.size(-1);
    const long long M = x.numel() / C;
    const int nslots = (int)(dsum.numel() / (2 * C));
    TORCH_CHECK(nslots >= 1 && dsum.numel() == (int64_t)nslots * 2 * C, "dsum must be [slots, 2, C]");
    if (zero_dsum) check(cudaMemsetAsync(dsum.data_ptr(), 0, sizeof(float) * dsum.numel(), cur_stream()), "bn_bwd/memset");
    check(rlr::launch_bn_bwd_reduce(bf(dy), nullptr, bf(x), f32(mean_rstd), f32(dsum), M, C, 2, num_sms(), cur_stream(),
                                    (const float*)gamma.data_ptr(), (const float*)beta.data_ptr(), nslots), "bn_bwd_reduce(recompute)");
    check(rlr::launch_bn_bwd_apply(bf(dy), nullptr, bf(x), (const float*)gamma.data_ptr(), f32(mean_rstd), f32(dsum), bfm(dx), nullptr,
                                   (float*)dgamma.data_ptr(), (float*)dbeta.data_ptr(), M, C, 2, num_sms(), cur_stream(),
                                   (const float*)beta.data_ptr(), nslots), "bn_bwd_apply(recompute)");
}
void gn_fwd(at::Tensor x, c10::optional<at::Tensor> res, at::Tensor y, at::Tensor gamma, at::Tensor beta, at::Tensor mean_rstd, int64_t groups,
            double eps, bool relu) {
    c10::cuda::CUDAGuard g(x.device());
    TORCH_CHECK(x.dim() == 4 && y.sizes() == x.sizes() && (!res.has_value() || !res->defined() || res->sizes() == x.sizes()), "gn_fwd: shapes");
    const int B = x.size(0), HW = x.size(1) * x.size(2), C = x.size(3);
    TORCH_CHECK(gamma.numel() == C && beta.numel() == C && mean_rstd.numel() == (int64_t)B * 2 * groups, "gn_fwd: gamma/beta [C], mean_rstd [B,2,groups]");
    check(rlr::launch_gn_fwd(bf(x), bfo(res), bfm(y), f32(gamma), f32(beta), f32(mean_rstd), B, HW, C, (int)groups, (float)eps, relu, num_sms(),
                             cur_stream()), "gn_fwd");
}
void gn_bwd(at::Tensor dy, c10::optional<at::Tensor> y, at::Tensor x, at::Tensor gamma, at::Tensor mean_rstd, at::Tensor dx,
            c10::optional<at::Tensor> dres, at::Tensor dgamma, at::Tensor dbeta, int64_t groups, bool relu) {
    c10::cuda::CUDAGuard g(x.device());
    TORCH_CHECK(x.dim() == 4 && dy.sizes() == x.sizes() && dx.sizes() == x.sizes(), "gn_bwd: shapes");
    TORCH_CHECK(!relu || (y.has_value() && y->defined() && y->sizes() == x.sizes()), "gn_bwd: relu needs the forward output y");
    TORCH_CHECK(!dres.has_value() || !dres->defined() || dres->sizes() == x.sizes(), "gn_bwd: dres shape");
    const int B = x.size(0), HW = x.size(1) * x.size(2), C = x.size(3);
    TORCH_CHECK(gamma.numel() == C && dgamma.numel() == C && dbeta.numel() == C && mean_rstd.numel() == (int64_t)B * 2 * groups,
                "gn_bwd: gamma/dgamma/dbeta [C], mean_rstd [B,2,groups]");
    check(rlr::launch_gn_bwd(bf(dy), relu ? bf(*y) : nullptr, bf(x), f32(gamma), f32(mean_rstd), bfm(dx), const_cast<__nv_bfloat16*>(bfo(dres)),
                             f32(dgamma), f32(dbeta), B, HW, C, (int)groups, relu, num_sms(), cur_stream()), "gn_bwd");
}
void relu_bwd(at::Tensor dy, at::Tensor y, double scale) {
    c10::cuda::CUDAGuard g(dy.device());
    check(rlr::launch_relu_bwd(bfm(dy), bf(y), dy.numel(), num_sms(), cur_stream(), (float)scale), "relu_bwd");
}
void maxpool2_fwd(at::Tensor x, at::Tensor y, at::Tensor idx, double drop_p, int64_t drop_seed, c10::optional<at::Tensor> drop_step, int64_t drop_stream) {
    c10::cuda::CUDAGuard g(x.device());
    const rlr::DropSpec d = drop_spec(drop_p, drop_seed, drop_step, drop_stream);
    check(rlr::launch_maxpool2_fwd(bf(x), bfm(y), (uint8_t*)idx.data_ptr(), x.size(0), x.size(1), x.size(2), x.size(3), cur_stream(),
                                   (float)drop_p, d.seed, d.step, d.stream), "maxpool2_fwd");
}
void maxpool2_bwd(at::Tensor dy, at::Tensor idx, at::Tensor dx, double drop_p, int64_t drop_seed, c10::optional<at::Tensor> drop_step, int64_t drop_stream,
                  c10::optional<at::Tensor> relu_out) {
    c10::cuda::CUDAGuard g(dx.device());
    const rlr::DropSpec d = drop_spec(drop_p, drop_seed, drop_step, drop_stream);
    const bool zm = relu_out.has_value() && relu_out->defined();
    TORCH_CHECK(!zm || (relu_out->scalar_type() == at::kBFloat16 && relu_out->is_contiguous() && relu_out->numel() == dy.numel()), "relu_out must match dy");
    TORCH_CHECK(dy.is_contiguous() && dx.is_contiguous() && idx.is_contiguous() && dy.size(1) == dx.size(1) / 2 && dy.size(2) == dx.size(2) / 2);
    check(rlr::launch_maxpool2_bwd(bf(dy), (const uint8_t*)idx.data_ptr(), bfm(dx), dx.size(0), dx.size(1), dx.size(2), dx.size(3), cur_stream(),
                                   (float)drop_p, d.seed, d.step, d.stream, zm ? bf(*relu_out) : nullptr), "maxpool2_bwd");
}
void avgpool_fwd(at::Tensor x, at::Tensor y) {
    c10::cuda::CUDAGuard g(x.device());
    check(rlr::launch_avgpool_fwd(bf(x), bfm(y), x.size(0), x.size(1) * x.size(2), x.size(3), cur_stream()), "avgpool_fwd");
}
void avgpool_bwd(at::Tensor dy, at::Tensor dx) {
    c10::cuda::CUDAGuard g(dx.device());
    check(rlr::launch_avgpool_bwd(bf(dy), bfm(dx), dx.size(0), dx.size(1) * dx.size(2), dx.size(3), cur_stream()), "avgpool_bwd");
}
void dropout_fwd(at::Tensor x, at::Tensor y, at::Tensor mask, double p, int64_t seed, at::Tensor step, int64_t stream) {
    c10::cuda::CUDAGuard g(x.device());
    check(rlr::launch_dropout_fwd(bf(x), bfm(y), (uint8_t*)mask.data_ptr(), x.numel(), (float)p, (uint64_t)seed,
                                  (const long long*)step.data_ptr(), (uint64_t)stream, cur_stream()), "dropout_fwd");
}
void dropout_bwd(at::Tensor dy, at::Tensor mask, at::Tensor dx, double p) {
    c10::cuda::CUDAGuard g(dx.device());
    check(rlr::launch_dropout_bwd(bf(dy), (const uint8_t*)mask.data_ptr(), bfm(dx), dx.numel(), (float)p, cur_stream()), "dropout_bwd");
}
void space_to_depth(at::Tensor x, at::Tensor y) {
    c10::cuda::CUDAGuard g(x.device());
    check(rlr::launch_space_to_depth(bf(x), bfm(y), x.size(0), x.size(1), x.size(2), x.size(3), num_sms(), cur_stream()), "space_to_depth");
}
void im2col_small(at::Tensor x, at::Tensor A, int64_t k, int64_t pad) {
    c10::cuda::CUDAGuard g(x.device());
    const int NB = x.size(0), H = x.size(1), W = x.size(2), C = x.size(3);
    const int Ho = H + 2 * pad - k + 1, Wo = W + 2 * pad - k + 1;
    TORCH_CHECK(x.dim() == 4 && x.is_contiguous() && A.is_contiguous() && A.numel() == (int64_t)NB * Ho * Wo * 64, "im2col_small: A must be [NB*Ho*Wo, 64]");
    check(rlr::launch_im2col_small(bf(x), bfm(A), NB, H, W, C, Ho, Wo, (int)k, (int)pad, num_sms(), cur_stream()), "im2col_small");
}
void depth_to_space(at::Tensor x4, at::Tensor y, bool accumulate, int64_t plane_mask) {
    c10::cuda::CUDAGuard g(y.device());
    check(rlr::launch_depth_to_space(bf(x4), bfm(y), y.size(0), y.size(1), y.size(2), y.size(3), accumulate, (int)plane_mask, num_sms(),
                                     cur_stream()), "depth_to_space");
}
void filter_gather_transpose(at::Tensor w, at::Tensor wt, int64_t Cout, int64_t T, int64_t Cin, std::vector<int64_t> taps) {
    c10::cuda::CUDAGuard g(w.device());
    int t[9];
    TORCH_CHECK(taps.size() >= 1 && taps.size() <= 9);
    for (size_t i = 0; i < taps.size(); ++i) t[i] = (int)taps[i];
    check(rlr::launch_filter_gather_transpose(bf(w), bfm(wt), Cout, T, Cin, (int)taps.size(), t, cur_stream()), "filter_gather_transpose");
}
void filter_transpose(at::Tensor w, at::Tensor wt, int64_t Cout, int64_t ntaps, int64_t Cin) {
    c10::cuda::CUDAGuard g(w.device());
    check(rlr::launch_filter_transpose(bf(w), bfm(wt), Cout, ntaps, Cin, cur_stream()), "filter_transpose");
}
void linear_small_fwd(at::Tensor x, at::Tensor w, c10::optional<at::Tensor> bias, at::Tensor y, bool relu) {
    c10::cuda::CUDAGuard g(x.device());
    check(rlr::launch_linear_small_fwd(bf(x), bf(w), opt<const float>(bias), bfm(y), x.size(0), x.size(1), w.size(0), relu, cur_stream()), "linear_small_fwd");
}
void linear_small_bwd(at::Tensor x, at::Tensor dy, at::Tensor w, c10::optional<at::Tensor> dx, at::Tensor dw, c10::optional<at::Tensor> db,
                      bool accumulate_dx) {
    c10::cuda::CUDAGuard g(x.device());
    check(rlr::launch_linear_small_bwd(bf(x), bf(dy), bf(w), const_cast<__nv_bfloat16*>(bfo(dx)), (float*)dw.data_ptr(), opt<float>(db),
                                       x.size(0), x.size(1), w.size(0), accumulate_dx, cur_stream()), "linear_small_bwd");
}
void linear_small_fwd2(at::Tensor x, at::Tensor w, c10::optional<at::Tensor> bias, at::Tensor y, bool relu) {
    c10::cuda::CUDAGuard g(x.device());
    check(rlr::launch_linear_small_fwd2(bf(x), bf(w), opt<const float>(bias), bfm(y), x.size(0), x.size(1), w.size(0), relu, cur_stream()), "linear_small_fwd2");
}
void linear_small_bwd2(at::Tensor x, at::Tensor dy, at::Tensor w, c10::optional<at::Tensor> dx, at::Tensor dw, c10::optional<at::Tensor> db,
                       bool accumulate_dx) {
    c10::cuda::CUDAGuard g(x.device());
    check(rlr::launch_linear_small_bwd2(bf(x), bf(dy), bf(w), const_cast<__nv_bfloat16*>(bfo(dx)), (float*)dw.data_ptr(), opt<float>(db),
                                        x.size(0), x.size(1), w.size(0), accumulate_dx, cur_stream()), "linear_small_bwd2");
}
}

void register_gemm_bindings(py::module_& m) {
    m.attr("STAT_SLOTS") = rlr::kStatSlots;
    m.def("set_persistent_conv", [](bool on) { rlr::set_persistent_conv(on ? 1 : 0); });
    m.def("set_pdl", [](bool on) { rlr::set_pdl(on ? 1 : 0); });
    m.def("set_conv_occ3", [](int64_t level) { rlr::set_conv_occ3((int)level); });
    m.def("set_conv_tma_store", [](bool on) { rlr::set_conv_tma_store(on ? 1 : 0); });
    m.def("set_conv_split_producer", [](bool on) { rlr::set_conv_split_producer(on ? 1 : 0); });
    m.def("set_conv_trace", [](c10::optional<at::Tensor> buf) {
        rlr::set_conv_trace(buf.has_value() && buf->defined() ? reinterpret_cast<long long*>(buf->data_ptr<int64_t>()) : nullptr);
    });
    m.def("gemm_bf16", &gemm_bf16, py::arg("A"), py::arg("B"), py::arg("out"), py::arg("bias"), py::arg("relu"), py::arg("accumulate"), py::arg("stats"),
          py::arg("drop_p") = 0.0, py::arg("drop_seed") = 0, py::arg("drop_step") = py::none(), py::arg("drop_stream") = 0);
    m.def("stem_gemm_bf16", &stem_gemm_bf16, py::arg("A"), py::arg("W"), py::arg("out"), py::arg("bias"), py::arg("relu"), py::arg("stats"),
          py::arg("ready_ptr") = 0, py::arg("lo") = 0, py::arg("hi") = 0, py::arg("epoch") = py::none());
    m.def("gemm_splitk_bf16", &gemm_splitk_bf16, py::arg("A"), py::arg("B"), py::arg("out"), py::arg("ws"), py::arg("bias"), py::arg("relu"),
          py::arg("drop_p") = 0.0, py::arg("drop_seed") = 0, py::arg("drop_step") = py::none(), py::arg("drop_stream") = 0);
    m.def("conv_bf16", &conv_bf16);
    m.def("conv_bf16_strided", &conv_bf16_strided);
    m.def("conv_wgrad_bf16_strided", &conv_wgrad_bf16_strided);
    m.def("conv3x3_halo_bf16", &conv3x3_halo_bf16);
    m.def("conv3x3_halo3_bf16", &conv3x3_halo3_bf16);
    m.def("conv_wgrad_bf16", &conv_wgrad_bf16);
    m.def("linear_wgrad_bf16", &linear_wgrad_bf16);
    m.def("conv_wgrad_halo_bf16", &conv_wgrad_halo_bf16);
    m.def("channel_stats", &channel_stats);
    m.def("ordered_sum", &ordered_sum);
    m.def("bias_grad", &bias_grad);
    m.def("bn_finalize", &bn_finalize);
    m.def("bn_apply", &bn_apply);
    m.def("bn_bwd", &bn_bwd);
    m.def("bn_bwd_recompute", &bn_bwd_recompute);
    m.def("gn_fwd", &gn_fwd);
    m.def("gn_bwd", &gn_bwd);
    m.def("relu_bwd", &relu_bwd, py::arg("dy"), py::arg("y"), py::arg("scale") = 1.0);
    m.def("maxpool2_fwd", &maxpool2_fwd, py::arg("x"), py::arg("y"), py::arg("idx"), py::arg("drop_p") = 0.0, py::arg("drop_seed") = 0,
          py::arg("drop_step") = py::none(), py::arg("drop_stream") = 0);
    m.def("maxpool2_bwd", &maxpool2_bwd, py::arg("dy"), py::arg("idx"), py::arg("dx"), py::arg("drop_p") = 0.0, py::arg("drop_seed") = 0,
          py::arg("drop_step") = py::none(), py::arg("drop_stream") = 0, py::arg("relu_out") = py::none());
    m.def("avgpool_fwd", &avgpool_fwd);
    m.def("avgpool_bwd", &avgpool_bwd);
    m.def("dropout_fwd", &dropout_fwd);
    m.def("dropout_bwd", &dropout_bwd);
    m.def("space_to_depth", &space_to_depth);
    m.def("im2col_small", &im2col_small);
    m.def("filter_transpose", &filter_transpose);
    m.def("depth_to_space", &depth_to_space);
    m.def("filter_gather_transpose", &filter_gather_transpose);
    m.def("linear_small_fwd", &linear_small_fwd);
    m.def("linear_small_bwd", &linear_small_bwd);
    m.def("linear_small_fwd2", &linear_small_fwd2);
    m.def("linear_small_bwd2", &linear_small_bwd2);
}
```

defending-against-backdoors-with-robust-learning-rate_b200/ops/nn.py:

```python
from __future__ import annotations

import math
import os

import torch
import torch.nn.functional as F

_scratch = {}
_s2d_done = {}
STAT_SLOTS = 16
USE_WGRAD_HALO = True
USE_STRIDED_TMA = bool(int(os.environ.get("RLR_STRIDED_TMA", "1")))
USE_IM2COL_STEM = bool(int(os.environ.get("RLR_IM2COL_STEM", "1")))
USE_BN_RECOMPUTE = bool(int(os.environ.get("RLR_BN_RECOMPUTE", "1")))
USE_HALO3 = bool(int(os.environ.get("RLR_HALO3", "0")))
USE_HALO_ANY = bool(int(os.environ.get("RLR_HALO_ANY", "1")))
USE_SPLITK = bool(int(os.environ.get("RLR_SPLITK", "1")))
USE_HEAD_V2 = bool(int(os.environ.get("RLR_HEAD_V2", "1")))


def _stem_ok(k, stride, cin, cout):
    return USE_IM2COL_STEM and stride == 1 and cin * k * k <= 64 and cout % 8 == 0 and (cout <= 64 or cout % 128 == 0)


def stem_geometry(in_shape, a):
    h, w, c = in_shape
    k, s, p = a["k"], a.get("stride", 1), a.get("pad", 0)
    if not _stem_ok(k, s, c, a["cout"]):
        return None
    return k, p, h + 2 * p - k + 1, w + 2 * p - k + 1


def _ext():
    from . import ext
    return ext()


def _zero(t):
    from . import zero_
    return zero_(t)


def _fallback(site, detail=""):
    from . import note_fallback
    note_fallback(site, detail)


def scratch(tag, shape, dtype, device):
    key = (tag, tuple(shape), dtype, str(device))
    t = _scratch.get(key)
    if t is None:
        t = _scratch[key] = torch.zeros(shape, dtype=dtype, device=device)
    return t


def conv_supported(in_shape, a, kind):
    h, w, cin = in_shape
    k, s, p, cout = a["k"], a.get("stride", 1), a.get("pad", 0), a["cout"]
    if k not in (1, 3) or s not in (1, 2) or cout % 8:
        return False
    even = s == 1 or (h % 2 == 0 and w % 2 == 0)
    if kind == "fwd":
        return even and (cin % 64 == 0 or cin < 64)
    if kind == "dgrad":
        return even and cin % 8 == 0 and cout % 64 == 0
    if kind == "wgrad":
        return even and (cin % 64 == 0 or cin < 64) and (cout <= 64 or cout % 128 == 0)
    return False


def _halo_ok(k, stride, pad, cin, h, w, stats=False):
    if not (k == 3 and stride == 1 and cin == 64 and pad in (0, 1, 2)):
        return False
    if not USE_HALO_ANY:
        return pad == 1 and h % 16 == 0 and w % 8 == 0
    ho, wo = h + 2 * pad - 2, w + 2 * pad - 2
    if ho < 1 or wo < 1:
        return False
    if stats and (ho % 16 or wo % 8):
        return False
    return 2 * ho * wo >= (-(-ho // 16) * 16) * (-(-wo // 8) * 8)


def _wgrad_halo_ok(k, stride, pad, cin, h, w):
    return k == 3 and stride == 1 and pad == 1 and cin == 64 and h % 16 == 0 and w % 8 == 0


def _taps(k, stride, pad):
    dh, dw, pl = [], [], []
    for dy in range(k):
        for dx in range(k):
            oy, ox = dy - pad, dx - pad
            if stride == 1:
                dh.append(oy); dw.append(ox); pl.append(0)
            else:
                dh.append(oy // 2); dw.append(ox // 2); pl.append((oy % 2) * 2 + (ox % 2))
    return dh, dw, pl


def conv2d_fwd_sm100(x, w, bias, y, stride, pad, relu, stats, tag="fwd", zero_stats=True, s2d_epoch=None, wait=None):
    e = _ext()
    Cout, k = w.shape[0], w.shape[1]
    if x.dim() == 2:
        B, Ho, Wo, Cin = y.shape[0], y.shape[1], y.shape[2], w.shape[3]
        assert x.shape == (B * Ho * Wo, 64) and _stem_ok(k, stride, Cin, Cout)
        if stats is not None and zero_stats:
            _zero(stats)
        rp, lo, hi, ep = wait if wait is not None else (0, 0, 0, None)
        e.stem_gemm_bf16(x, w.reshape(Cout, k * k * Cin), y.view(B * Ho * Wo, Cout), bias, bool(relu), stats, int(rp), int(lo), int(hi), ep)
        return y
    B, H, W, Cin = x.shape
    if _stem_ok(k, stride, Cin, Cout):
        Ho, Wo = y.shape[1], y.shape[2]
        A = scratch(("im2col", tag), (B * Ho * Wo, 64), x.dtype, x.device)
        e.im2col_small(x.contiguous(), A, k, pad)
        if stats is not None and zero_stats:
            _zero(stats)
        e.stem_gemm_bf16(A, w.reshape(Cout, k * k * Cin), y.view(B * Ho * Wo, Cout), bias, bool(relu), stats, 0, 0, 0, None)
        return y
    if Cin % 64:
        cp = (Cin + 63) // 64 * 64
        xp = scratch(("xpad", tag), (B, H, W, cp), x.dtype, x.device)
        e.pad_rows(x.reshape(B * H * W, Cin), xp.view(B * H * W, cp))
        wp = scratch(("wpad", tag, w.data_ptr()), (Cout, k, k, cp), w.dtype, w.device)
        e.pad_rows(w.reshape(Cout * k * k, Cin), wp.view(Cout * k * k, cp))
        x, w, Cin = xp, wp, cp
    if _halo_ok(k, stride, pad, Cin, H, W, stats is not None):
        if USE_HALO3 and stats is None and pad == 1 and H % 16 == 0:
            e.conv3x3_halo3_bf16(x, w.reshape(Cout, 9 * 64), y, bias, bool(relu), False)
            return y
        if stats is not None and zero_stats:
            _zero(stats)
        e.conv3x3_halo_bf16(x, w.reshape(Cout, 9 * 64), y, bias, bool(relu), False, stats, 0, None)
        return y
    if stride == 2 and USE_STRIDED_TMA and stats is None:
        e.conv_bf16_strided(x, w.reshape(Cout, k * k * Cin), y, [dy_ - pad for dy_ in range(k) for _ in range(k)],
                            [dx_ - pad for _ in range(k) for dx_ in range(k)], bias, bool(relu), False, [], 0, 2, 1, 0, 0)
        return y
    planes = 1
    if stride == 2:
        key = ("s2d", x.data_ptr(), Cin)
        x4 = scratch(key, (4 * B, H // 2, W // 2, Cin), x.dtype, x.device)
        if s2d_epoch is None or _s2d_done.get(key + (B,)) != s2d_epoch:
            e.space_to_depth(x, x4)
            _s2d_done[key + (B,)] = s2d_epoch
        x, planes = x4, 4
    dh, dw, pl = _taps(k, stride, pad)
    if stats is not None and zero_stats:
        _zero(stats)
    e.conv_bf16(x, w.reshape(Cout, k * k * Cin), y, B, planes, dh, dw, pl, bias, bool(relu), False, stats, [], 0)
    return y


def conv2d_dgrad_sm100(dy, w, dx, stride, pad, accumulate):
    e = _ext()
    Cout, k, _, Cin = w.shape
    B = dy.shape[0]
    if stride == 2:
        return _conv2d_dgrad_s2(e, dy, w, dx, pad, accumulate)
    if _halo_ok(k, 1, k - 1 - pad, Cout, dy.shape[1], dy.shape[2]) and dx.shape[-1] % 8 == 0:
        wt = scratch(("wt", w.data_ptr(), dx.data_ptr()), (Cin, k * k * Cout), w.dtype, w.device)
        e.filter_transpose(w, wt, Cout, k * k, Cin)
        if USE_HALO3 and pad == 1 and dy.shape[1] % 16 == 0:
            e.conv3x3_halo3_bf16(dy, wt, dx, None, False, bool(accumulate))
        else:
            e.conv3x3_halo_bf16(dy, wt, dx, None, False, bool(accumulate), None, 0, None)
        return dx
    dh, dw, pl = _taps(k, 1, k - 1 - pad)
    if Cin % 64 == 0:
        T = k * k
        e.conv_bf16(dy, w.reshape(Cout, T * Cin), dx, B, 1, dh, dw, pl, None, False, bool(accumulate), None,
                    [T - 1 - t for t in range(T)], T)
        return dx
    wt = scratch(("wt", w.data_ptr(), dx.data_ptr()), (Cin, k * k * Cout), w.dtype, w.device)
    e.filter_transpose(w, wt, Cout, k * k, Cin)
    e.conv_bf16(dy, wt, dx, B, 1, dh, dw, pl, None, False, bool(accumulate), None, [], 0)
    return dx


def _conv2d_dgrad_s2(e, dy, w, dx, pad, accumulate):
    Cout, k, _, Cin = w.shape
    B, Ho, Wo, _ = dy.shape
    plan = []
    for pi in range(2):
        for pj in range(2):
            taps, dh, dw = [], [], []
            for fy in range(k):
                for fx in range(k):
                    if (pi + pad - fy) % 2 == 0 and (pj + pad - fx) % 2 == 0:
                        taps.append(fy * k + fx); dh.append((pi + pad - fy) // 2); dw.append((pj + pad - fx) // 2)
            if taps:
                plan.append((pi, pj, taps, dh, dw))
    if USE_STRIDED_TMA and Cin % 64 == 0 and dx.shape[1] == 2 * Ho and dx.shape[2] == 2 * Wo:
        if not accumulate and len(plan) < 4:
            _zero(dx)
        for pi, pj, taps, dh, dw in plan:
            e.conv_bf16_strided(dy, w.reshape(Cout, k * k * Cin), dx, dh, dw, None, False, bool(accumulate), taps, k * k, 1, 2, pi, pj)
        return dx
    dx4 = scratch(("dx4", w.data_ptr(), dx.data_ptr()), (4 * B, Ho, Wo, Cin), dy.dtype, dy.device)
    mask = 0
    for pi, pj, taps, dh, dw in plan:
        plane = pi * 2 + pj
        mask |= 1 << plane
        if Cin % 64 == 0:
            e.conv_bf16(dy, w.reshape(Cout, k * k * Cin), dx4[plane * B:(plane + 1) * B], B, 1, dh, dw, [0] * len(taps), None,
                        False, False, None, taps, k * k)
            continue
        wt = scratch(("wt_s2", w.data_ptr(), dx.data_ptr(), plane), (Cin, len(taps) * Cout), w.dtype, w.device)
        e.filter_gather_transpose(w, wt, Cout, k * k, Cin, taps)
        e.conv_bf16(dy, wt, dx4[plane * B:(plane + 1) * B], B, 1, dh, dw, [0] * len(taps), None, False, False, None, [], 0)
    e.depth_to_space(dx4, dx, bool(accumulate), mask)
    return dx


def conv2d_wgrad_sm100(x, dy, gw, gb, stride, pad, tag="fwd", zero=True):
    e = _ext()
    Cout, k = gw.shape[0], gw.shape[1]
    pre = x.dim() == 2
    B, H, W, Cin = (dy.shape[0], 0, 0, gw.shape[3]) if pre else x.shape
    cin_valid = Cin
    if pre or _stem_ok(k, stride, Cin, Cout):
        Ho, Wo = dy.shape[1], dy.shape[2]
        A = x if pre else scratch(("im2col", tag), (B * Ho * Wo, 64), x.dtype, x.device)
        dW = scratch(("dwstem", tag), (Cout, 64), torch.float32, x.device)
        _zero(dW)
        e.linear_wgrad_bf16(dy.view(B * Ho * Wo, Cout), A, dW)
        if zero:
            _zero(gw)
        e.unpad_add(dW, gw.view(Cout, k * k * Cin))
        if gb is not None:
            _bias_grad(e, dy, gb, zero)
        return
    if Cin % 64:
        cp = (Cin + 63) // 64 * 64
        x = scratch(("xpad", tag), (B, H, W, cp), x.dtype, x.device)
        Cin = cp
    planes = 1
    strided = stride == 2 and USE_STRIDED_TMA
    if stride == 2 and not strided:
        x = scratch(("s2d", x.data_ptr(), Cin), (4 * B, H // 2, W // 2, Cin), x.dtype, x.device)
        planes = 4
    dh, dw, pl = _taps(k, stride, pad)
    if zero:
        _zero(gw)
    if strided:
        e.conv_wgrad_bf16_strided(dy, x, gw, cin_valid, [dy_ - pad for dy_ in range(k) for _ in range(k)],
                                  [dx_ - pad for _ in range(k) for dx_ in range(k)], 2)
    elif USE_WGRAD_HALO and _wgrad_halo_ok(k, stride, pad, Cin, H, W) and (Cout <= 64 or Cout % 128 == 0):
        e.conv_wgrad_halo_bf16(dy, x, gw, cin_valid)
    else:
        e.conv_wgrad_bf16(dy, x, gw, B, planes, cin_valid, dh, dw, pl)
    if gb is not None:
        _bias_grad(e, dy, gb, zero)


def _bias_ok(C):
    return C >= 8 and C <= 2048 and C % 8 == 0 and 256 % (C // 8) == 0


def _bias_grad(e, dy, gb, zero):
    C = dy.shape[-1]
    if zero:
        _zero(gb)
    if _bias_ok(C):
        e.bias_grad(dy.contiguous(), gb)
    else:
        _fallback("bias_grad", f"C={C}")
        gb.add_(dy.float().reshape(-1, C).sum(0))


def bn_fwd(x, y, res, gamma, beta, rm, rv, stats, mean_rstd, count, eps, momentum, train, relu, impl, stats_buf=None):
    C = x.shape[-1]
    if impl == "sm100":
        e = _ext()
        if train and stats is None:
            if stats_buf is not None:
                stats = stats_buf
            else:
                stats = scratch(("bnstats", mean_rstd.data_ptr()), (1, 2, C), torch.float32, x.device)
                _zero(stats)
            e.channel_stats(x, stats)
        e.bn_apply(x, res, y, gamma, beta, mean_rstd, bool(relu), 1 if train else 2, stats if train else None, float(count), float(eps),
                   float(momentum), rm, rv)
        return
    xf = x.float().reshape(-1, C)
    if train:
        if stats is not None:
            tot = stats.reshape(-1, 2, C).sum(0)
            mean = tot[0] / count
            var = (tot[1] / count - mean * mean).clamp_min(0)
        else:
            mean = xf.mean(0)
            var = xf.var(0, unbiased=False)
        rm.mul_(1 - momentum).add_(momentum * mean)
        rv.mul_(1 - momentum).add_(momentum * var * (count / max(1, count - 1)))
        mean_rstd[0].copy_(mean); mean_rstd[1].copy_(torch.rsqrt(var + eps))
    else:
        mean_rstd[0].copy_(rm); mean_rstd[1].copy_(torch.rsqrt(rv + eps))
    out = (xf - mean_rstd[0]) * (mean_rstd[1] * gamma) + beta
    if res is not None:
        out = out + res.float().reshape(-1, C)
    if relu:
        out = out.clamp_min(0)
    y.copy_(out.reshape(y.shape))


def bn_bwd(dy, y, x, gamma, mean_rstd, dsum, dx, dres, dgamma, dbeta, relu, impl, zero_dsum=True, beta=None):
    C = x.shape[-1]
    if impl == "sm100":
        if USE_BN_RECOMPUTE and relu and dres is None and beta is not None:
            _ext().bn_bwd_recompute(dy, x, gamma, beta, mean_rstd, dsum, dx, dgamma, dbeta, bool(zero_dsum))
            return
        _ext().bn_bwd(dy, y, x, gamma, mean_rstd, dsum, dx, dres, dgamma, dbeta, bool(relu), bool(zero_dsum))
        return
    dz = dy.float().reshape(-1, C)
    if relu:
        dz = dz * (y.float().reshape(-1, C) > 0)
    if dres is not None:
        dres.copy_(dz.reshape(dres.shape))
    xhat = (x.float().reshape(-1, C) - mean_rstd[0]) * mean_rstd[1]
    s0, s1 = dz.sum(0), (dz * xhat).sum(0)
    M = dz.shape[0]
    dbeta.copy_(s0); dgamma.copy_(s1)
    dx.copy_((gamma * mean_rstd[1] * (dz - s0 / M - xhat * s1 / M)).reshape(dx.shape))


def gn_supported(x, groups):
    C = x.shape[-1]
    cpg = C // groups if groups > 0 and C % groups == 0 else 0
    return x.dim() == 4 and C % 8 == 0 and cpg > 0 and (8 // math.gcd(8, cpg)) * cpg <= 2048


def gn_fwd(x, y, res, gamma, beta, mean_rstd, groups, eps, relu, impl):
    if impl == "sm100":
        if gn_supported(x, groups):
            _ext().gn_fwd(x, res, y, gamma, beta, mean_rstd, int(groups), float(eps), bool(relu))
            return
        _fallback("gn_fwd", f"shape={tuple(x.shape)} groups={groups}")
    B, C = x.shape[0], x.shape[-1]
    xg = x.float().reshape(B, -1, groups, C // groups)
    mean = xg.mean((1, 3))
    var = xg.var((1, 3), unbiased=False)
    rstd = torch.rsqrt(var + eps)
    mean_rstd[:, 0].copy_(mean); mean_rstd[:, 1].copy_(rstd)
    out = ((xg - mean[:, None, :, None]) * rstd[:, None, :, None]).reshape(B, -1, C) * gamma + beta
    if res is not None:
        out = out + res.float().reshape(B, -1, C)
    if relu:
        out = out.clamp_min(0)
    y.copy_(out.reshape(y.shape))


def gn_bwd(dy, y, x, gamma, mean_rstd, dx, dres, dgamma, dbeta, groups, relu, impl, zero=True):
    if zero:
        _zero(dgamma)
        _zero(dbeta)
    if impl == "sm100":
        if gn_supported(x, groups):
            _ext().gn_bwd(dy, y if relu else None, x, gamma, mean_rstd, dx, dres, dgamma, dbeta, int(groups), bool(relu))
            return
        _fallback("gn_bwd", f"shape={tuple(x.shape)} groups={groups}")
    B, C = x.shape[0], x.shape[-1]
    G, cpg = groups, C // groups
    dz = dy.float().reshape(B, -1, C)
    if relu:
        dz = dz * (y.float().reshape(B, -1, C) > 0)
    if dres is not None:
        dres.copy_(dz.reshape(dres.shape))
    mean, rstd = mean_rstd[:, 0], mean_rstd[:, 1]
    xhat = ((x.float().reshape(B, -1, G, cpg) - mean[:, None, :, None]) * rstd[:, None, :, None]).reshape(B, -1, C)
    dgamma.add_((dz * xhat).sum((0, 1)))
    dbeta.add_(dz.sum((0, 1)))
    dzg = (dz * gamma).reshape(B, -1, G, cpg)
    M = dzg.shape[1] * cpg
    s_a = dzg.sum((1, 3))[:, None, :, None]
    s_b = (dzg * xhat.reshape(B, -1, G, cpg)).sum((1, 3))[:, None, :, None]
    d = rstd[:, None, :, None] * (dzg - s_a / M - xhat.reshape(B, -1, G, cpg) * s_b / M)
    dx.copy_(d.reshape(dx.shape))


def relu_bwd_(dy, y, impl, scale=1.0):
    if impl == "sm100" and dy.numel() % 8 == 0:
        _ext().relu_bwd(dy, y, float(scale))
    else:
        if impl == "sm100":
            _fallback("relu_bwd", f"numel={dy.numel()}")
        dy.mul_((y > 0).to(dy.dtype) * scale)


def maxpool2_fwd(x, y, idx, impl, drop=None, mask=None):
    if impl == "sm100" and x.shape[-1] % 8 == 0:
        if drop is not None:
            _ext().maxpool2_fwd(x, y, idx, float(drop[0]), int(drop[1]), drop[2], int(drop[3]))
        else:
            _ext().maxpool2_fwd(x, y, idx)
        return
    if impl == "sm100":
        _fallback("maxpool2_fwd", f"C={x.shape[-1]}")
    B, H, W, C = x.shape
    Ho, Wo = H // 2, W // 2
    win = x[:, :Ho * 2, :Wo * 2].reshape(B, Ho, 2, Wo, 2, C).permute(0, 1, 3, 5, 2, 4).reshape(B, Ho, Wo, C, 4)
    v, i = win.float().max(-1)
    if drop is not None:
        keep = torch.rand(v.shape, device=v.device) >= drop[0]
        mask.copy_(keep)
        v = v * keep / (1 - drop[0])
    y.copy_(v); idx.copy_(i)


def maxpool2_bwd(dy, idx, dx, impl, drop=None, mask=None, relu_out=None):
    if impl == "sm100" and dx.shape[-1] % 8 == 0:
        kw = dict(relu_out=relu_out.contiguous()) if relu_out is not None else {}
        if drop is not None:
            _ext().maxpool2_bwd(dy, idx, dx, float(drop[0]), int(drop[1]), drop[2], int(drop[3]), **kw)
        else:
            _ext().maxpool2_bwd(dy, idx, dx, **kw)
        return
    if impl == "sm100":
        _fallback("maxpool2_bwd", f"C={dx.shape[-1]}")
    if relu_out is not None:
        dy = dy * (relu_out > 0).to(dy.dtype)
    B, H, W, C = dx.shape
    Ho, Wo = H // 2, W // 2
    dx.zero_()
    if drop is not None:
        dy = dy * mask.to(dy.dtype) / (1 - drop[0])
    oh = F.one_hot(idx.long(), 4).to(dy.dtype) * dy.unsqueeze(-1)
    dx[:, :Ho * 2, :Wo * 2].copy_(oh.reshape(B, Ho, Wo, C, 2, 2).permute(0, 1, 4, 2, 5, 3).reshape(B, Ho * 2, Wo * 2, C))


def avgpool_fwd(x, y, impl):
    if impl == "sm100":
        _ext().avgpool_fwd(x, y)
    else:
        y.copy_(x.float().mean((1, 2), keepdim=True))


def avgpool_bwd(dy, dx, impl):
    if impl == "sm100":
        _ext().avgpool_bwd(dy, dx)
    else:
        dx.copy_((dy.float() / (dx.shape[1] * dx.shape[2])).expand_as(dx))


def dropout_fwd(x, y, mask, p, seed, step, stream, impl):
    if impl == "sm100" and x.numel() % 8 == 0:
        _ext().dropout_fwd(x, y, mask, float(p), int(seed), step, int(stream))
        return
    if impl == "sm100":
        _fallback("dropout_fwd", f"numel={x.numel()}")
    keep = torch.rand(x.shape, device=x.device) >= p
    mask.copy_(keep)
    y.copy_(x * keep / (1 - p))


def dropout_bwd(dy, mask, dx, p, impl):
    if impl == "sm100" and dx.numel() % 8 == 0:
        _ext().dropout_bwd(dy, mask, dx, float(p))
    else:
        if impl == "sm100":
            _fallback("dropout_bwd", f"numel={dx.numel()}")
        dx.copy_(dy * mask / (1 - p))


def linear_fused_dropout_ok(N, K):
    return N > 32 and K % 64 == 0 and N % 64 == 0


def linear_fwd(x, w, bias, y, relu, impl, drop=None):
    N, K = w.shape
    dk = dict(drop_p=float(drop[0]), drop_seed=int(drop[1]), drop_step=drop[2], drop_stream=int(drop[3])) if drop is not None else {}
    if impl == "sm100":
        if N <= 32:
            if USE_HEAD_V2 and K % 2 == 0 and (N * K) % 8 == 0 and N * K * 2 <= 48 * 1024:
                _ext().linear_small_fwd2(x.contiguous(), w, bias, y, bool(relu))
                return
            _ext().linear_small_fwd(x.contiguous(), w, bias, y, bool(relu))
            return
        if K % 64 == 0 and N % 64 == 0:
            M = x.shape[0]
            if USE_SPLITK and K >= 1024 and ((M + 127) // 128) * ((N + 127) // 128) <= 16:
                ws = scratch(("splitk_ws", y.data_ptr()), (M, N), torch.float32, x.device)
                _ext().gemm_splitk_bf16(x.contiguous(), w, y, ws, bias, bool(relu), **dk)
                return
            _ext().gemm_bf16(x.contiguous(), w, y, bias, bool(relu), False, None, **dk)
            return
        _fallback("linear_fwd", f"N={N} K={K}")
    out = F.linear(x, w.to(x.dtype), bias.to(x.dtype) if bias is not None else None)
    if relu:
        out = F.relu(out)
    if drop is not None:
        out = out * (torch.rand(out.shape, device=out.device) >= drop[0]) / (1 - drop[0])
    y.copy_(out)


def linear_bwd(x, dy, w, dx, dw, db, acc_dx, impl, zero=True):
    N, K = w.shape
    if impl == "sm100" and N <= 32:
        if USE_HEAD_V2 and K % 2 == 0:
            if zero:
                _zero(dw)
                if db is not None:
                    _zero(db)
            _ext().linear_small_bwd2(x.contiguous(), dy.contiguous(), w, dx, dw, db, bool(acc_dx))
            return
        _ext().linear_small_bwd(x.contiguous(), dy.contiguous(), w, dx, dw, db, bool(acc_dx))
        return
    dyf = dy.to(x.dtype)
    sm = impl == "sm100" and K % 64 == 0 and N % 64 == 0
    if sm and (N <= 64 or N % 128 == 0):
        if zero:
            _zero(dw)
        _ext().linear_wgrad_bf16(dy.contiguous(), x.contiguous(), dw)
    else:
        if impl == "sm100":
            _fallback("linear_wgrad", f"N={N} K={K}")
        dw.copy_(dyf.t() @ x)
    if db is not None:
        if sm and _bias_ok(N):
            _bias_grad(_ext(), dy, db, zero)
        else:
            if impl == "sm100":
                _fallback("linear_bias_grad", f"N={N}")
            db.copy_(dyf.float().sum(0))
    if dx is not None:
        if sm:
            wt = scratch(("wt_lin", w.data_ptr(), dx.data_ptr()), (K, N), w.dtype, w.device)
            _ext().filter_transpose(w, wt, N, 1, K)
            _ext().gemm_bf16(dy.contiguous(), wt, dx, None, False, bool(acc_dx), None)
            return
        if impl == "sm100":
            _fallback("linear_dgrad", f"N={N} K={K}")
        d = dyf @ w.to(x.dtype)
        if acc_dx:
            dx.add_(d)
        else:
            dx.copy_(d)
```

Baseline: 0.6158.

## Fuse stride-2 dgrad phase planes and shortcut 1x1 dgrad into one grouped launch

```diff
diff --git a/defending-against-backdoors-with-robust-learning-rate_b200/models/native.py b/defending-against-backdoors-with-robust-learning-rate_b200/models/native.py
--- a/defending-against-backdoors-with-robust-learning-rate_b200/models/native.py
+++ b/defending-against-backdoors-with-robust-learning-rate_b200/models/native.py
@@ -203,6 +203,17 @@
             if op.need_dx:
                 op.acc_dx = op.x in written
                 written.add(op.x)
+        for op in plan:
+            a = op.attrs
+            if not (op.kind == "conv" and op.need_dx and op.acc_dx and a.get("stride", 1) == 2 and a["k"] == 3 and a.get("pad", 0) == 1):
+                continue
+            writers = [q for q in plan if (q.need_dx and q.x == op.x) or q.res == op.x]
+            sc = next((q for q in writers if q is not op), None)
+            if (len(writers) != 2 or sc is None or sc.kind != "conv" or sc.res == op.x or sc.acc_dx or sc.attrs.get("stride", 1) != 2
+                    or sc.attrs["k"] != 1 or sc.attrs.get("pad", 0) != 0 or sc.attrs["cout"] != a["cout"]):
+                continue
+            op.saved["dgrad_pair"] = sc
+            sc.saved["dgrad_by"] = op
 
     def _numel(self, shp):
         return int(math.prod(shp))
@@ -390,11 +401,25 @@
             gw.copy_(dw.permute(0, 2, 3, 1))
             if gb is not None:
                 gb.copy_(db)
-        if not op.need_dx:
+        if not op.need_dx or "dgrad_by" in op.saved:
             return
         dx = self.G(op.x, B)
+        sc = op.saved.get("dgrad_pair")
+        if sc is not None:
+            dy_sc, w_sc = self.G(sc.y, B), self.pwb[sc.name + ".weight"]
+            if (self.impl["conv_dgrad"] == "sm100" and ops.conv_supported(op.in_shape, a, "dgrad")
+                    and ops.conv_supported(sc.in_shape, sc.attrs, "dgrad")):
+                ops.conv2d_dgrad_sm100(dy, self.pwb[name], dx, s, p, sc.acc_dx, shortcut=(dy_sc, w_sc))
+                return
+            self._dgrad(sc, x, dy_sc, dx, sc.acc_dx)
+        self._dgrad(op, x, dy, dx, op.acc_dx)
+
+    def _dgrad(self, op, x, dy, dx, acc):
+        a = op.attrs
+        name = op.name + ".weight"
+        s, p = a.get("stride", 1), a.get("pad", 0)
         if self.impl["conv_dgrad"] == "sm100" and ops.conv_supported(op.in_shape, a, "dgrad"):
-            ops.conv2d_dgrad_sm100(dy, self.pwb[name], dx, s, p, op.acc_dx)
+            ops.conv2d_dgrad_sm100(dy, self.pwb[name], dx, s, p, acc)
             return
         if self.impl["conv_dgrad"] == "sm100":
             ops.note_fallback("conv_dgrad", f"{op.name} in={op.in_shape} {a}")
@@ -402,7 +427,7 @@
             dy.permute(0, 3, 1, 2), x.permute(0, 3, 1, 2), self.pwb[name].permute(0, 3, 1, 2), None, [s, s], [p, p], [1, 1],
             False, [0, 0], 1, [True, False, False])
         di = di.permute(0, 2, 3, 1)
-        if op.acc_dx:
+        if acc:
             dx.add_(di)
         else:
             dx.copy_(di)
diff --git a/defending-against-backdoors-with-robust-learning-rate_b200/ops/csrc/gemm.cu b/defending-against-backdoors-with-robust-learning-rate_b200/ops/csrc/gemm.cu
--- a/defending-against-backdoors-with-robust-learning-rate_b200/ops/csrc/gemm.cu
+++ b/defending-against-backdoors-with-robust-learning-rate_b200/ops/csrc/gemm.cu
@@ -40,17 +40,29 @@
 };
 static_assert(sizeof(SharedTail) <= 640, "the bias slice starts 640 bytes into the tail");
 
-template <int BN, bool kStats, bool kBMN, int kOcc = 2>
+template <int BN, bool kStats, bool kBMN, int kOcc = 2, bool kGroup = false>
 __global__ void __launch_bounds__(kThreads, kOcc)
 umma_conv_gemm_kernel(const __grid_constant__ CUtensorMap tmA, const __grid_constant__ CUtensorMap tmB, const __grid_constant__ CUtensorMap tmC,
-                       const ConvGemmParams p) {
+                       const __grid_constant__ CUtensorMap tmA2, const __grid_constant__ CUtensorMap tmB2, const ConvGemmParams p) {
+    static_assert(!kGroup || (kBMN && !kStats), "plane-grouped launches are data gradients");
     using Cfg = TileCfg<BN, kOcc>;
     extern __shared__ uint8_t smem_raw[];
     uint8_t* smem = reinterpret_cast<uint8_t*>((reinterpret_cast<uintptr_t>(smem_raw) + 1023) & ~uintptr_t(1023));
     SharedTail* tail = reinterpret_cast<SharedTail*>(smem + Cfg::kRingBytes);
 
     const int warp = threadIdx.x >> 5, lane = threadIdx.x & 31;
-    const int tile_m = blockIdx.x, tile_n = blockIdx.y;
+    int tile_m = blockIdx.x, tile_n = blockIdx.y;
+    int num_kb = p.num_kb, tap0 = 0, sc_kb = 0, out_ph = p.out_ph, out_pw = p.out_pw;
+    if constexpr (kGroup) {
+        const int per_group = p.grp_mtiles * p.grp_ntiles;
+        const int g = blockIdx.x / per_group, rest = blockIdx.x - g * per_group;
+        tile_n = rest / p.grp_mtiles;
+        tile_m = rest - tile_n * p.grp_mtiles;
+        tap0 = p.grp_tap0[g];
+        num_kb = (p.grp_tap0[g + 1] - tap0) * p.cblocks;
+        sc_kb = g == p.sc_group ? p.cblocks : 0;
+        out_ph = p.grp_ph[g]; out_pw = p.grp_pw[g];
+    }
     long long* dbg = p.dbg ? p.dbg + ((size_t)blockIdx.y * gridDim.x + blockIdx.x) * 8 : nullptr;
     if (dbg && threadIdx.x == 0) { dbg[0] = (long long)gtimer(); uint32_t sm; asm volatile("mov.u32 %0, %%smid;" : "=r"(sm)); dbg[7] = sm; }
 
@@ -66,6 +78,7 @@
         prefetch_tmap(&tmA);
         prefetch_tmap(&tmB);
         if (p.tma_store) prefetch_tmap(&tmC);
+        if (kGroup && sc_kb) { prefetch_tmap(&tmA2); prefetch_tmap(&tmB2); }
         for (int s = 0; s < Cfg::kStages; ++s) { mbar_init(&tail->full[s], (p.split_prod || p.b_src) ? 2 : 1); mbar_init(&tail->empty[s], 8); }
         fence_barrier_init();
     }
@@ -75,7 +88,7 @@
         if (p.mode == 1) {
             const int tw = r % p.TW, th = (r / p.TW) % p.TH, tn = r / (p.TW * p.TH);
             const int w = w0 + tw, h = h0 + th, n = n0 + tn;
-            gi = (w < p.Wo && h < p.Ho && n < p.NB) ? ((n * p.OutH + h * p.out_stride + p.out_ph) * p.OutW + w * p.out_stride + p.out_pw) : -1;
+            gi = (w < p.Wo && h < p.Ho && n < p.NB) ? ((n * p.OutH + h * p.out_stride + out_ph) * p.OutW + w * p.out_stride + out_pw) : -1;
         } else {
             gi = tile_m * BM + r;
             if (gi >= p.M) gi = -1;
@@ -98,14 +111,18 @@
         } else if (lane == 0) {
             int stage = 0;
             uint32_t phase = 0;
-            for (int kb = 0; kb < p.num_kb; ++kb) {
+            for (int kb = 0; kb < sc_kb + num_kb; ++kb) {
                 mbar_wait(&tail->empty[stage], phase ^ 1);
                 uint8_t* sa = smem + stage * Cfg::kStageBytes;
                 uint8_t* sb = sa + Cfg::kABytes;
                 mbar_expect_tx(&tail->full[stage], p.split_prod ? Cfg::kABytes : Cfg::kStageBytes);
                 if (dbg && kb == 0) dbg[2] = (long long)gtimer();
-                if (p.mode == 1) {
-                    const int tap = kb / p.cblocks, cb = kb - tap * p.cblocks;
+                const bool sc = kGroup && kb < sc_kb;
+                int tap = 0, cb = kb;
+                if (p.mode == 1 && !sc) { tap = tap0 + (kb - sc_kb) / p.cblocks; cb = kb - sc_kb - (tap - tap0) * p.cblocks; }
+                if (sc) {
+                    tma_load_4d(&tmA2, &tail->full[stage], sa, cb * BK, w0, h0, n0);
+                } else if (p.mode == 1) {
                     tma_load_4d(&tmA, &tail->full[stage], sa, cb * BK, w0 * p.in_stride + p.dw[tap], h0 * p.in_stride + p.dh[tap],
                                 n0 + p.dn[tap]);
                 } else {
@@ -113,9 +130,9 @@
                 }
                 if (p.split_prod) {
                 } else if (kBMN) {
-                    const int tap = kb / p.cblocks, cb = kb - tap * p.cblocks;
                     for (int g = 0; g < BN / 64; ++g)
-                        tma_load_2d(&tmB, &tail->full[stage], sb + g * 8192, p.wtap[tap] * p.wcols + tile_n * BN + g * 64, cb * BK);
+                        tma_load_2d(sc ? &tmB2 : &tmB, &tail->full[stage], sb + g * 8192, (sc ? 0 : p.wtap[tap]) * p.wcols + tile_n * BN + g * 64,
+                                    cb * BK);
                 } else {
                     tma_load_2d(&tmB, &tail->full[stage], sb, kb * BK, tile_n * BN);
                 }
@@ -126,14 +143,16 @@
         if (p.split_prod && lane == 0) {
             int stage = 0;
             uint32_t phase = 0;
-            for (int kb = 0; kb < p.num_kb; ++kb) {
+            for (int kb = 0; kb < sc_kb + num_kb; ++kb) {
                 mbar_wait(&tail->empty[stage], phase ^ 1);
                 uint8_t* sb = smem + stage * Cfg::kStageBytes + Cfg::kABytes;
                 mbar_expect_tx(&tail->full[stage], Cfg::kBBytes);
                 if (kBMN) {
-                    const int tap = kb / p.cblocks, cb = kb - tap * p.cblocks;
+                    const bool sc = kGroup && kb < sc_kb;
+                    const int kc = kb - sc_kb, tap = sc ? 0 : tap0 + kc / p.cblocks, cb = sc ? kb : kc - (tap - tap0) * p.cblocks;
                     for (int g = 0; g < BN / 64; ++g)
-                        tma_load_2d(&tmB, &tail->full[stage], sb + g * 8192, p.wtap[tap] * p.wcols + tile_n * BN + g * 64, cb * BK);
+                        tma_load_2d(sc ? &tmB2 : &tmB, &tail->full[stage], sb + g * 8192, (sc ? 0 : p.wtap[tap]) * p.wcols + tile_n * BN + g * 64,
+                                    cb * BK);
                 } else {
                     tma_load_2d(&tmB, &tail->full[stage], sb, kb * BK, tile_n * BN);
                 }
@@ -154,8 +173,32 @@
         {
             int stage = 0;
             uint32_t phase = 0;
+            if constexpr (kGroup) {
+                if (sc_kb) {
+                    consumer_mainloop<BN, Cfg::kStages, Cfg::kStageBytes, Cfg::kABytes, kBMN>(
+                        acc, smem, tail->full, tail->empty, sc_kb, (uint32_t)wgi * 64 * 128, 0u, stage, phase, lane);
+                    const int r0 = wgi * 64 + frag_row(t, 0);
+#pragma unroll
+                    for (int h = 0; h < 2; ++h) {
+                        const int gi = tail->row_index[r0 + 8 * h];
+                        if (gi < 0) continue;
+                        uint32_t* row = reinterpret_cast<uint32_t*>(reinterpret_cast<__nv_bfloat16*>(p.out) + (size_t)gi * p.ldc + col0);
+#pragma unroll
+                        for (int j = 0; j < BN / 8; ++j) {
+                            const int c = frag_col(t, 4 * j);
+                            uint32_t v = pack_bf16x2(acc[4 * j + 2 * h], acc[4 * j + 2 * h + 1]);
+                            if (p.accumulate) {
+                                const float2 a = __bfloat1622float2(*reinterpret_cast<const __nv_bfloat162*>(&v));
+                                const float2 o = __bfloat1622float2(*reinterpret_cast<const __nv_bfloat162*>(row + c / 2));
+                                v = pack_bf16x2(a.x + o.x, a.y + o.y);
+                            }
+                            row[c / 2] = v;
+                        }
+                    }
+                }
+            }
             consumer_mainloop<BN, Cfg::kStages, Cfg::kStageBytes, Cfg::kABytes, kBMN>(
-                acc, smem, tail->full, tail->empty, p.num_kb, (uint32_t)wgi * 64 * 128, p.b_src ? smem_u32(smem + Cfg::kABytes) : 0u,
+                acc, smem, tail->full, tail->empty, num_kb, (uint32_t)wgi * 64 * 128, p.b_src ? smem_u32(smem + Cfg::kABytes) : 0u,
                 stage, phase, lane);
         }
         if (dbg && et == 0) dbg[4] = (long long)gtimer();
@@ -172,7 +215,9 @@
             for (int i = et; i < 2 * BN; i += kEpiThreads) red[i] = 0.f;
             named_bar(1, kEpiThreads);
         }
-        const bool tma_out = !kStats && p.tma_store;
+        const bool tma_out = !kStats && !kGroup && p.tma_store;
+        const bool rmw = kGroup ? (p.accumulate || p.pair || sc_kb > 0) : (bool)p.accumulate;
+        const bool load_old = kGroup ? (p.accumulate || sc_kb > 0) : (bool)p.accumulate;
 #pragma unroll
         for (int j = 0; j < BN / 8; ++j) {
             const int c = frag_col(t, 4 * j);
@@ -255,13 +300,13 @@
 #pragma unroll
         for (int it0 = 0; it0 < kIters; it0 += kBatch) {
             uint4 oldv[kBatch];
-            if (p.accumulate) {
+            if (rmw) {
 #pragma unroll
                 for (int j = 0; j < kBatch; ++j) {
                     const int idx = et + (it0 + j) * kEpiThreads, r = idx / kChunks, ch = idx - r * kChunks;
                     const int gi = tail->row_index[r];
                     oldv[j] = make_uint4(0, 0, 0, 0);
-                    if (gi >= 0 && col0 + ch * 8 < p.N) oldv[j] = *reinterpret_cast<const uint4*>(out + (size_t)gi * p.ldc + col0 + ch * 8);
+                    if (load_old && gi >= 0 && col0 + ch * 8 < p.N) oldv[j] = *reinterpret_cast<const uint4*>(out + (size_t)gi * p.ldc + col0 + ch * 8);
                 }
             }
 #pragma unroll
@@ -270,7 +315,7 @@
                 const int gi = tail->row_index[r];
                 if (gi < 0 || col0 + ch * 8 >= p.N) continue;
                 uint4 val = *reinterpret_cast<const uint4*>(staging + r * Cfg::kPitch + ch * 16);
-                if (p.accumulate) {
+                if (rmw) {
                     const __nv_bfloat162* o2 = reinterpret_cast<const __nv_bfloat162*>(&oldv[j]);
                     __nv_bfloat162* v2 = reinterpret_cast<__nv_bfloat162*>(&val);
 #pragma unroll
@@ -348,8 +393,8 @@
         configured = true;
     }
     dim3 grid(m_tiles, (p.N + BN - 1) / BN);
-    if (p.b_mn) return launch_kernel(umma_conv_gemm_kernel<BN, false, true, 3>, grid, dim3(kThreads), Cfg::kSmemBytes, st, tmA, tmB, tmC, p);
-    return launch_kernel(umma_conv_gemm_kernel<BN, false, false, 3>, grid, dim3(kThreads), Cfg::kSmemBytes, st, tmA, tmB, tmC, p);
+    if (p.b_mn) return launch_kernel(umma_conv_gemm_kernel<BN, false, true, 3>, grid, dim3(kThreads), Cfg::kSmemBytes, st, tmA, tmB, tmC, tmA, tmB, p);
+    return launch_kernel(umma_conv_gemm_kernel<BN, false, false, 3>, grid, dim3(kThreads), Cfg::kSmemBytes, st, tmA, tmB, tmC, tmA, tmB, p);
 }
 
 static int sm_count() {
@@ -377,6 +422,10 @@
 
 static int g_split_prod = -1;
 void set_conv_split_producer(int on) { g_split_prod = on ? 1 : 0; }
+static bool split_producer() {
+    if (g_split_prod < 0) { const char* e = getenv("RLR_SPLIT_PRODUCER"); g_split_prod = (e && atoi(e) == 0) ? 0 : 1; }
+    return g_split_prod != 0;
+}
 static long long* g_trace = nullptr;
 void set_conv_trace(long long* buf) { g_trace = buf; }
 long long* conv_trace_buf() { return g_trace; }
@@ -414,8 +463,7 @@
     p.tma_store = 0;
     if (tma_store_enabled() && !p.accumulate && ((reinterpret_cast<uintptr_t>(p.out) & 15) == 0) && make_out_tmap(&tmC, p) == cudaSuccess)
         p.tma_store = 1;
-    if (g_split_prod < 0) { const char* e = getenv("RLR_SPLIT_PRODUCER"); g_split_prod = (e && atoi(e) == 0) ? 0 : 1; }
-    p.split_prod = (g_split_prod && !p.b_src) ? 1 : 0;
+    p.split_prod = (split_producer() && !p.b_src) ? 1 : 0;
     if (p.b_src && !p.stats && p.N <= BN) {
         static const int stem_persistent = [] { const char* e = getenv("RLR_STEM_PERSISTENT"); return e ? atoi(e) : 2; }();
         if (stem_persistent && m_tiles >= 2 * sm_count())
@@ -433,9 +481,9 @@
         configured = true;
     }
     dim3 grid(m_tiles, (p.N + BN - 1) / BN);
-    if (p.b_mn) return launch_kernel(umma_conv_gemm_kernel<BN, false, true>, grid, dim3(kThreads), Cfg::kSmemBytes, st, tmA, tmB, tmC, p);
-    if (p.stats && !p.tma_store) return launch_kernel(umma_conv_gemm_kernel<BN, true, false>, grid, dim3(kThreads), Cfg::kSmemBytes, st, tmA, tmB, tmC, p);
-    return launch_kernel(umma_conv_gemm_kernel<BN, false, false>, grid, dim3(kThreads), Cfg::kSmemBytes, st, tmA, tmB, tmC, p);
+    if (p.b_mn) return launch_kernel(umma_conv_gemm_kernel<BN, false, true>, grid, dim3(kThreads), Cfg::kSmemBytes, st, tmA, tmB, tmC, tmA, tmB, p);
+    if (p.stats && !p.tma_store) return launch_kernel(umma_conv_gemm_kernel<BN, true, false>, grid, dim3(kThreads), Cfg::kSmemBytes, st, tmA, tmB, tmC, tmA, tmB, p);
+    return launch_kernel(umma_conv_gemm_kernel<BN, false, false>, grid, dim3(kThreads), Cfg::kSmemBytes, st, tmA, tmB, tmC, tmA, tmB, p);
 }
 
 static int pick_bn(int N) { return (N % 128 == 0) ? 128 : 64; }
@@ -491,6 +539,23 @@
 
 static int pow2_ceil(int x) { int p = 1; while (p < x) p <<= 1; return p; }
 
+static int conv_pick_bn(int NB, int Ho, int Wo, int Cout) {
+    int bn = pick_bn(Cout);
+    static const int small_bn64 = [] { const char* e = getenv("RLR_SMALL_BN64"); return e ? atoi(e) : 1; }();
+    const long long px = (long long)NB * Ho * Wo;
+    if (small_bn64 && bn == 128 && ((px + BM - 1) / BM) * (Cout / 128) < sm_count()) bn = 64;
+    return bn;
+}
+
+static int conv_tiles(ConvGemmParams& p, int NB, int Ho, int Wo) {
+    int TW = pow2_ceil(Wo); if (TW > BM) TW = BM;
+    int TH = pow2_ceil(Ho); if (TW * TH > BM) TH = BM / TW;
+    const int TN = BM / (TW * TH);
+    p.TW = TW; p.TH = TH; p.TN = TN;
+    p.tiles_w = (Wo + TW - 1) / TW; p.tiles_h = (Ho + TH - 1) / TH;
+    return p.tiles_w * p.tiles_h * ((NB + TN - 1) / TN);
+}
+
 cudaError_t launch_conv_bf16(const void* x, const void* w, void* out, int NB, int planes, int Hin, int Win, int Cin, int Ho, int Wo,
                              int Cout, int ldc, int ntaps, const int* dh, const int* dw, const int* dplane, const float* bias,
                              int relu, int accumulate, float* stats, cudaStream_t st, const int* wtap, int w_taps_total,
@@ -498,20 +563,10 @@
     if (Cin % BK || Cout % 8 || ntaps < 1 || ntaps > 9) return cudaErrorInvalidValue;
     if (in_stride < 1 || in_stride > 2 || out_stride < 1 || out_stride > 2 || (in_stride > 1 && planes != 1)) return cudaErrorInvalidValue;
     if (wtap && (stats || Cout % 64)) return cudaErrorInvalidValue;
-    int bn = pick_bn(Cout);
+    const int bn = conv_pick_bn(NB, Ho, Wo, Cout);
     ConvGemmParams p{};
-    {
-        static const int small_bn64 = [] { const char* e = getenv("RLR_SMALL_BN64"); return e ? atoi(e) : 1; }();
-        const long long px = (long long)NB * Ho * Wo;
-        if (small_bn64 && bn == 128 && ((px + BM - 1) / BM) * (Cout / 128) < sm_count()) bn = 64;
-    }
-    int TW = pow2_ceil(Wo); if (TW > BM) TW = BM;
-    int TH = pow2_ceil(Ho); if (TW * TH > BM) TH = BM / TW;
-    int TN = BM / (TW * TH);
-    p.TW = TW; p.TH = TH; p.TN = TN;
-    p.tiles_w = (Wo + TW - 1) / TW; p.tiles_h = (Ho + TH - 1) / TH;
-    const int tiles_n = (NB + TN - 1) / TN;
-    const int m_tiles = p.tiles_w * p.tiles_h * tiles_n;
+    const int m_tiles = conv_tiles(p, NB, Ho, Wo);
+    const int TW = p.TW, TH = p.TH, TN = p.TN;
     p.M = NB * Ho * Wo; p.N = Cout; p.mode = 1; p.cblocks = Cin / BK; p.num_kb = ntaps * p.cblocks; p.ntaps = ntaps;
     p.Ho = Ho; p.Wo = Wo; p.NB = NB;
     p.in_stride = in_stride; p.out_stride = out_stride; p.out_ph = out_ph; p.out_pw = out_pw; p.OutH = Ho * out_stride; p.OutW = Wo * out_stride;
@@ -542,4 +597,73 @@
     return bn == 128 ? launch_bn<128>(tmA, tmB, p, m_tiles, st) : launch_bn<64>(tmA, tmB, p, m_tiles, st);
 }
 
-}
+template <int BN, int kOcc>
+static cudaError_t launch_group_bn(const CUtensorMap& tmA, const CUtensorMap& tmB, const CUtensorMap& tmA2, const CUtensorMap& tmB2,
+                                   const ConvGemmParams& p, int groups, cudaStream_t st) {
+    using Cfg = TileCfg<BN, kOcc>;
+    static bool configured = false;
+    if (!configured) {
+        RLR_CUDA_CHECK(cudaFuncSetAttribute(umma_conv_gemm_kernel<BN, false, true, kOcc, true>, cudaFuncAttributeMaxDynamicSharedMemorySize,
+                                            Cfg::kSmemBytes));
+        configured = true;
+    }
+    ConvGemmParams q = p;
+    q.grp_ntiles = p.N / BN;
+    const dim3 grid(groups * q.grp_ntiles * q.grp_mtiles, 1);
+    return launch_kernel(umma_conv_gemm_kernel<BN, false, true, kOcc, true>, grid, dim3(kThreads), Cfg::kSmemBytes, st, tmA, tmB, tmA, tmA2, tmB2, q);
+}
+
+cudaError_t launch_conv_dgrad_s2_bf16(const void* dy, const void* w, void* dx, const void* dy_sc, const void* w_sc, int NB, int Ho, int Wo,
+                                      int Cout, int Cin, int k, int accumulate, cudaStream_t st) {
+    if ((k != 1 && k != 3) || Cout % BK || Cin % 64 || NB < 1 || Ho < 1 || Wo < 1) return cudaErrorInvalidValue;
+    if (dy_sc && (k != 3 || !w_sc)) return cudaErrorInvalidValue;
+    const int pad = k == 3 ? 1 : 0;
+    const int bn = conv_pick_bn(NB, Ho, Wo, Cin);
+    ConvGemmParams p{};
+    p.grp_mtiles = conv_tiles(p, NB, Ho, Wo);
+    p.M = NB * Ho * Wo; p.N = Cin; p.mode = 1; p.cblocks = Cout / BK; p.Ho = Ho; p.Wo = Wo; p.NB = NB;
+    p.in_stride = 1; p.out_stride = 2; p.OutH = 2 * Ho; p.OutW = 2 * Wo;
+    p.out = dx; p.ldc = Cin; p.accumulate = accumulate; p.b_mn = 1; p.wcols = Cin;
+    p.dbg = g_trace; p.tma_store = 0; p.split_prod = split_producer() ? 1 : 0;
+    p.sc_group = -1; p.pair = dy_sc ? 1 : 0;
+    static const int order[4][2] = {{1, 1}, {0, 1}, {1, 0}, {0, 0}};
+    int groups = 0, T = 0;
+    for (const auto& pl : order) {
+        const int pi = pl[0], pj = pl[1], first = T;
+        for (int fy = 0; fy < k; ++fy)
+            for (int fx = 0; fx < k; ++fx)
+                if ((pi + pad - fy) % 2 == 0 && (pj + pad - fx) % 2 == 0) {
+                    p.dh[T] = (int8_t)((pi + pad - fy) / 2); p.dw[T] = (int8_t)((pj + pad - fx) / 2); p.dn[T] = 0; p.wtap[T] = fy * k + fx;
+                    ++T;
+                }
+        if (T == first && accumulate) continue;
+        p.grp_tap0[groups] = first; p.grp_ph[groups] = pi; p.grp_pw[groups] = pj;
+        if (dy_sc && pi == 0 && pj == 0) p.sc_group = groups;
+        ++groups;
+    }
+    p.grp_tap0[groups] = T;
+    p.ntaps = T;
+    CUtensorMap tmA, tmB, tmA2, tmB2;
+    {
+        const uint64_t d[4] = {(uint64_t)Cout, (uint64_t)Wo, (uint64_t)Ho, (uint64_t)NB};
+        const uint64_t s[3] = {(uint64_t)Cout * 2, (uint64_t)Wo * Cout * 2, (uint64_t)Ho * Wo * Cout * 2};
+        const uint32_t b[4] = {BK, (uint32_t)p.TW, (uint32_t)p.TH, (uint32_t)p.TN};
+        RLR_CUDA_CHECK(make_tmap_bf16(&tmA, dy, 4, d, s, b));
+        tmA2 = tmA;
+        if (dy_sc) RLR_CUDA_CHECK(make_tmap_bf16(&tmA2, dy_sc, 4, d, s, b));
+    }
+    {
+        const uint64_t cols = (uint64_t)k * k * Cin;
+        const uint64_t d[2] = {cols, (uint64_t)Cout}, s[1] = {cols * 2};
+        const uint32_t b[2] = {64, BK};
+        RLR_CUDA_CHECK(make_tmap_bf16(&tmB, w, 2, d, s, b));
+        tmB2 = tmB;
+        const uint64_t d1[2] = {(uint64_t)Cin, (uint64_t)Cout}, s1[1] = {(uint64_t)Cin * 2};
+        if (dy_sc) RLR_CUDA_CHECK(make_tmap_bf16(&tmB2, w_sc, 2, d1, s1, b));
+    }
+    if (bn == 128) return launch_group_bn<128, 2>(tmA, tmB, tmA2, tmB2, p, groups, st);
+    if (conv_occ3() >= 1) return launch_group_bn<64, 3>(tmA, tmB, tmA2, tmB2, p, groups, st);
+    return launch_group_bn<64, 2>(tmA, tmB, tmA2, tmB2, p, groups, st);
+}
+
+}
diff --git a/defending-against-backdoors-with-robust-learning-rate_b200/ops/csrc/gemm.h b/defending-against-backdoors-with-robust-learning-rate_b200/ops/csrc/gemm.h
--- a/defending-against-backdoors-with-robust-learning-rate_b200/ops/csrc/gemm.h
+++ b/defending-against-backdoors-with-robust-learning-rate_b200/ops/csrc/gemm.h
@@ -24,6 +24,9 @@
     int b_mn;
     int wtap[9];
     int wcols;
+    int grp_mtiles, grp_ntiles, sc_group, pair;
+    int grp_tap0[5];
+    int grp_ph[4], grp_pw[4];
     DropSpec drop;
     int tma_store;
     int split_prod;
@@ -59,6 +62,8 @@
                              int Cout, int ldc, int ntaps, const int* dh, const int* dw, const int* dplane, const float* bias,
                              int relu, int accumulate, float* stats, cudaStream_t st, const int* wtap = nullptr, int w_taps_total = 0,
                              int in_stride = 1, int out_stride = 1, int out_ph = 0, int out_pw = 0);
+cudaError_t launch_conv_dgrad_s2_bf16(const void* dy, const void* w, void* dx, const void* dy_sc, const void* w_sc, int NB, int Ho, int Wo,
+                                      int Cout, int Cin, int k, int accumulate, cudaStream_t st);
 
 cudaError_t launch_conv3x3_halo_bf16(const void* x, const void* w, void* out, int NB, int Hin, int Win, int H, int W, int Cout, const float* bias,
                                      int relu, int accumulate, float* stats, int bo_mode, long long* dbg, int num_sms, cudaStream_t st);
diff --git a/defending-against-backdoors-with-robust-learning-rate_b200/ops/csrc/gemm_binding.cpp b/defending-against-backdoors-with-robust-learning-rate_b200/ops/csrc/gemm_binding.cpp
--- a/defending-against-backdoors-with-robust-learning-rate_b200/ops/csrc/gemm_binding.cpp
+++ b/defending-against-backdoors-with-robust-learning-rate_b200/ops/csrc/gemm_binding.cpp
@@ -110,6 +110,27 @@
     check(rlr::launch_conv_bf16(bf(x), bf(w), bfm(out), NB, 1, Hin, Win, Cin, Ho, Wo, Cout, Cout, T, a, b, c, opt<const float>(bias), relu,
                                 accumulate, nullptr, cur_stream(), bmn ? wt : nullptr, (int)w_taps_total, (int)in_stride, (int)out_stride,
                                 (int)out_ph, (int)out_pw), "conv_bf16_strided");
+}
+
+void conv_dgrad_s2_bf16(at::Tensor dy, at::Tensor w, at::Tensor dx, c10::optional<at::Tensor> dy_sc, c10::optional<at::Tensor> w_sc,
+                        bool accumulate) {
+    c10::cuda::CUDAGuard g(dy.device());
+    TORCH_CHECK(dy.dim() == 4 && w.dim() == 4 && dx.dim() == 4, "conv_dgrad_s2: dy, w, dx must be 4-D");
+    const int NB = dy.size(0), Ho = dy.size(1), Wo = dy.size(2), Cout = dy.size(3), k = w.size(1), Cin = dx.size(3);
+    TORCH_CHECK(k == 1 || k == 3, "conv_dgrad_s2: 3x3 (pad 1) or 1x1 (pad 0) filters");
+    TORCH_CHECK(w.size(0) == Cout && w.size(2) == k && w.size(3) == Cin, "conv_dgrad_s2: filter must be [Cout,k,k,Cin]");
+    TORCH_CHECK(dx.size(0) == NB && dx.size(1) == 2 * Ho && dx.size(2) == 2 * Wo, "conv_dgrad_s2: dx must be [NB,2Ho,2Wo,Cin]");
+    TORCH_CHECK(Cin % 64 == 0 && Cout % 64 == 0, "conv_dgrad_s2: Cin and Cout must be multiples of 64");
+    const bool sc = dy_sc.has_value() && dy_sc->defined();
+    TORCH_CHECK(sc == (w_sc.has_value() && w_sc->defined()), "conv_dgrad_s2: dy_sc and w_sc go together");
+    if (sc) {
+        TORCH_CHECK(k == 3, "conv_dgrad_s2: the shortcut pairs with a 3x3 conv");
+        TORCH_CHECK(dy_sc->sizes() == dy.sizes(), "conv_dgrad_s2: dy_sc must have dy's shape");
+        TORCH_CHECK(w_sc->dim() == 4 && w_sc->size(0) == Cout && w_sc->size(1) == 1 && w_sc->size(2) == 1 && w_sc->size(3) == Cin,
+                    "conv_dgrad_s2: w_sc must be [Cout,1,1,Cin]");
+    }
+    check(rlr::launch_conv_dgrad_s2_bf16(bf(dy), bf(w), bfm(dx), sc ? bf(*dy_sc) : nullptr, sc ? bf(*w_sc) : nullptr, NB, Ho, Wo, Cout, Cin, k,
+                                         accumulate, cur_stream()), "conv_dgrad_s2_bf16");
 }
 
 void conv3x3_halo_bf16(at::Tensor x, at::Tensor w, at::Tensor out, c10::optional<at::Tensor> bias, bool relu, bool accumulate,
@@ -372,6 +393,7 @@
           py::arg("drop_p") = 0.0, py::arg("drop_seed") = 0, py::arg("drop_step") = py::none(), py::arg("drop_stream") = 0);
     m.def("conv_bf16", &conv_bf16);
     m.def("conv_bf16_strided", &conv_bf16_strided);
+    m.def("conv_dgrad_s2_bf16", &conv_dgrad_s2_bf16);
     m.def("conv_wgrad_bf16_strided", &conv_wgrad_bf16_strided);
     m.def("conv3x3_halo_bf16", &conv3x3_halo_bf16);
     m.def("conv3x3_halo3_bf16", &conv3x3_halo3_bf16);
diff --git a/defending-against-backdoors-with-robust-learning-rate_b200/ops/nn.py b/defending-against-backdoors-with-robust-learning-rate_b200/ops/nn.py
--- a/defending-against-backdoors-with-robust-learning-rate_b200/ops/nn.py
+++ b/defending-against-backdoors-with-robust-learning-rate_b200/ops/nn.py
@@ -152,12 +152,13 @@
     return y
 
 
-def conv2d_dgrad_sm100(dy, w, dx, stride, pad, accumulate):
+def conv2d_dgrad_sm100(dy, w, dx, stride, pad, accumulate, shortcut=None):
     e = _ext()
     Cout, k, _, Cin = w.shape
     B = dy.shape[0]
     if stride == 2:
-        return _conv2d_dgrad_s2(e, dy, w, dx, pad, accumulate)
+        return _conv2d_dgrad_s2(e, dy, w, dx, pad, accumulate, shortcut)
+    assert shortcut is None, "only stride-2 data gradients pair with a shortcut"
     if _halo_ok(k, 1, k - 1 - pad, Cout, dy.shape[1], dy.shape[2]) and dx.shape[-1] % 8 == 0:
         wt = scratch(("wt", w.data_ptr(), dx.data_ptr()), (Cin, k * k * Cout), w.dtype, w.device)
         e.filter_transpose(w, wt, Cout, k * k, Cin)
@@ -178,9 +179,20 @@
     return dx
 
 
-def _conv2d_dgrad_s2(e, dy, w, dx, pad, accumulate):
+def _conv2d_dgrad_s2(e, dy, w, dx, pad, accumulate, shortcut=None):
     Cout, k, _, Cin = w.shape
     B, Ho, Wo, _ = dy.shape
+    strided = USE_STRIDED_TMA and Cin % 64 == 0 and dx.shape[1] == 2 * Ho and dx.shape[2] == 2 * Wo
+    if shortcut is not None:
+        assert k == 3 and pad == 1 and shortcut[1].shape[1:3] == (1, 1), "a 3x3/p1 conv pairs with a 1x1/p0 shortcut"
+    fused = getattr(e, "conv_dgrad_s2_bf16", None) if strided and (k, pad) in ((3, 1), (1, 0)) else None
+    if fused is not None:
+        dy_sc, w_sc = shortcut if shortcut is not None else (None, None)
+        fused(dy, w, dx, dy_sc, w_sc, bool(accumulate))
+        return dx
+    if shortcut is not None:
+        _conv2d_dgrad_s2(e, shortcut[0], shortcut[1], dx, 0, accumulate)
+        accumulate = True
     plan = []
     for pi in range(2):
         for pj in range(2):
@@ -191,7 +203,7 @@
                         taps.append(fy * k + fx); dh.append((pi + pad - fy) // 2); dw.append((pj + pad - fx) // 2)
             if taps:
                 plan.append((pi, pj, taps, dh, dw))
-    if USE_STRIDED_TMA and Cin % 64 == 0 and dx.shape[1] == 2 * Ho and dx.shape[2] == 2 * Wo:
+    if strided:
         if not accumulate and len(plan) < 4:
             _zero(dx)
         for pi, pj, taps, dh, dw in plan:
```

New measurement: 0.6294 (median of 6 runs). 1.02x the previous value.
